# adamjorr/kbbq-py

Measured on NVIDIA B200. Metric: bases/sec recalibrated (table build + apply), higher is better.
Workload: dtype u8 in/out, u32->int64 counts, f64 model

## Files before the change

include/kbbq_b200.h:

```cpp
#ifndef KBBQ_B200_H
#define KBBQ_B200_H

#include <stddef.h>
#include <stdint.h>

#ifdef __cplusplus
extern "C" {
#endif

#define KBBQ_NQ 43
#define KBBQ_NDINUC 16

#define KBBQ_OK 0
#define KBBQ_E_ARG (-1)
#define KBBQ_E_CUDA (-2)
#define KBBQ_E_WORKSPACE (-3)
#define KBBQ_E_DATA (-4)
#define KBBQ_E_IO (-5)
#define KBBQ_E_FORMAT (-6)
#define KBBQ_E_RAGGED (-7)
#define KBBQ_E_NAME_FIELD (-8)
#define KBBQ_E_NAME_RG (-9)
#define KBBQ_E_NAME_MISMATCH (-10)
#define KBBQ_E_PEER (-11)
#define KBBQ_E_UNSUPPORTED (-12)

#define KBBQ_FLAG_QUAL_RANGE 1
#define KBBQ_FLAG_BAD_BASE 2
#define KBBQ_FLAG_RG_RANGE 4
#define KBBQ_FLAG_SEGMENTS 8
#define KBBQ_FLAG_KMER_FULL 16

int kbbq_abi_version(void);
const char *kbbq_strerror(int code);
const char *kbbq_last_cuda_error(void);

int64_t kbbq_pos_table_elems(int L, int R);
int64_t kbbq_din_table_elems(int R);

int kbbq_workspace_bytes(int64_t N, int L, int R, size_t *bytes);

int kbbq_build(const uint8_t *seq_dev, const uint8_t *qual_dev, const uint8_t *corr_dev,
               const uint16_t *rg_dev, const uint8_t *second_dev, int64_t N, int L, int R,
               int minscore, int64_t *pos_errs_dev, int64_t *pos_total_dev, int64_t *din_errs_dev,
               int64_t *din_total_dev, void *workspace_dev, size_t workspace_bytes,
               int *status_dev, int path, void *stream);

int kbbq_marginals(const int64_t *pos_errs_dev, const int64_t *pos_total_dev, int L, int R,
                   int64_t *q_errs_dev, int64_t *q_total_dev, int64_t *rg_errs_dev,
                   int64_t *rg_total_dev, int64_t *meanq_dev, void *stream);

int kbbq_delta_q(const int64_t *prior_q_dev, const int64_t *numerrs_dev,
                 const int64_t *numtotal_dev, int64_t n, int64_t *delta_dev, void *stream);

int kbbq_posterior_q_real(const double *prior_q_dev, const int64_t *numerrs_dev,
                          const int64_t *numtotal_dev, int64_t n, int64_t *posterior_dev, void *stream);

int kbbq_bam_workspace_bytes(int64_t N, int L, int R, size_t *bytes);
int kbbq_build_bam(const uint8_t *seq_dev, const uint8_t *qual_dev, const uint8_t *err_dev,
                   const uint8_t *skip_dev, const uint16_t *rg_dev, const uint8_t *flags_dev,
                   const uint16_t *aln_start_dev, const uint16_t *aln_end_dev, int64_t N, int L, int R,
                   int minscore, int64_t *pos_errs_dev, int64_t *pos_total_dev, int64_t *din_errs_dev,
                   int64_t *din_total_dev, void *workspace_dev, size_t workspace_bytes, int *status_dev,
                   void *stream);
int kbbq_apply_bam(const uint8_t *seq_dev, const uint8_t *qual_dev, const uint16_t *rg_dev,
                   const uint8_t *flags_dev, int64_t N, int L, int R, int minscore,
                   const int64_t *meanq_dev, const int64_t *rgdq_dev, const int64_t *qdq_dev,
                   const int64_t *posdq_dev, const int64_t *dindq_dev, int nq, int ndin1,
                   uint8_t *out_qual_dev, void *workspace_dev, size_t workspace_bytes, int *status_dev,
                   void *stream);

int kbbq_calibration_counts(const uint8_t *qual_dev, const uint8_t *err_dev, const uint8_t *seq_dev,
                            const uint8_t *corr_dev, const uint8_t *skip_dev, int64_t n,
                            int64_t *total_dev, int64_t *errs_dev, void *stream);

int kbbq_get_delta_qs(const int64_t *meanq_dev, const int64_t *rg_errs_dev,
                      const int64_t *rg_total_dev, const int64_t *q_errs_dev,
                      const int64_t *q_total_dev, const int64_t *pos_errs_dev,
                      const int64_t *pos_total_dev, const int64_t *din_errs_dev,
                      const int64_t *din_total_dev, int R, int nq, int ncyc, int ndin,
                      int64_t *rgdq_dev, int64_t *qdq_dev, int64_t *posdq_dev, int64_t *dindq_dev,
                      void *stream);

#define KBBQ_APPLY_BASES_CHECKED 0x10
int kbbq_apply(const uint8_t *seq_dev, const uint8_t *qual_dev, const uint16_t *rg_dev,
               const uint8_t *second_dev, int64_t N, int L, int R, int minscore,
               const int64_t *meanq_dev, const int64_t *rgdq_dev, const int64_t *qdq_dev,
               const int64_t *posdq_dev, const int64_t *dindq_dev, int nq, int ndin1,
               uint8_t *out_qual_dev, void *workspace_dev, size_t workspace_bytes, int *status_dev,
               int path, void *stream);

int64_t kbbq_segment_rows_bound(int64_t N, int R);
int64_t kbbq_segment_table_elems(int R);
int kbbq_segmented_supported(int L, int R, int minscore);
int kbbq_segment_plan(const uint16_t *rg_dev, const uint8_t *second_dev, int64_t N, int R, uint32_t *seg_dev,
                      uint32_t *dest_dev, int *status_dev, void *stream);
int kbbq_segment_rows(const uint8_t *src_dev, const uint32_t *dest_dev, int64_t N, int L, uint8_t *dst_segmented_dev,
                      void *stream);
int kbbq_segment_pad(const uint32_t *seg_dev, int R, int L, uint8_t *seq_dev, uint8_t *qual_dev, uint8_t *corr_dev,
                     void *stream);
int kbbq_unsegment_rows(const uint8_t *src_segmented_dev, const uint32_t *dest_dev, int64_t N, int L,
                        int64_t rows_bound, uint8_t *dst_dev, void *stream);
int kbbq_build_segmented(const uint8_t *seq_dev, const uint8_t *qual_dev, const uint8_t *corr_dev,
                         const uint32_t *seg_dev, int64_t rows_bound, int L, int R, int minscore,
                         int64_t *pos_errs_dev, int64_t *pos_total_dev, int64_t *din_errs_dev,
                         int64_t *din_total_dev, void *workspace_dev, size_t workspace_bytes, int *status_dev,
                         void *stream);
int kbbq_apply_segmented(const uint8_t *seq_dev, const uint8_t *qual_dev, const uint32_t *seg_dev, int64_t rows_bound,
                         int L, int R, int minscore, const int64_t *meanq_dev, const int64_t *rgdq_dev,
                         const int64_t *qdq_dev, const int64_t *posdq_dev, const int64_t *dindq_dev, int nq,
                         int ndin1, uint8_t *out_qual_dev, void *workspace_dev, size_t workspace_bytes,
                         int *status_dev, void *stream);
int kbbq_apply_segmented_flags(const uint8_t *seq_dev, const uint8_t *qual_dev, const uint32_t *seg_dev,
                               int64_t rows_bound, int L, int R, int minscore, const int64_t *meanq_dev,
                               const int64_t *rgdq_dev, const int64_t *qdq_dev, const int64_t *posdq_dev,
                               const int64_t *dindq_dev, int nq, int ndin1, uint8_t *out_qual_dev, void *workspace_dev,
                               size_t workspace_bytes, int *status_dev, int flags, void *stream);

int kbbq_recalibrate_host(const uint8_t *seq, const uint8_t *qual, const uint8_t *corr,
                          const uint16_t *rg, const uint8_t *second, int64_t N, int L, int R,
                          int minscore, uint8_t *out_qual, int64_t *tables_host,
                          int64_t *deltas_host, int *status_out, int device);
int kbbq_recalibrate_host_multi(const uint8_t *seq, const uint8_t *qual, const uint8_t *corr,
                                const uint16_t *rg, const uint8_t *second, int64_t N, int L, int R,
                                int minscore, uint8_t *out_qual, int64_t *tables_host,
                                int64_t *deltas_host, int *status_out, const int *devices, int n_dev);

int kbbq_recalibrate_fastq(const char *reads_path, const char *corrected_path, int infer_rg, int minscore, int out_fd,
                           int device, int threads, int64_t *n_reads, int *n_rg, int *status_out);

int kbbq_host_release(int device);
int kbbq_host_last_traffic(int device, int64_t *h2d_bytes, int64_t *d2h_bytes);
int kbbq_host_pack_mode(int host_threads);

typedef struct kbbq_session kbbq_session;
int kbbq_session_create(int device, int L, int R, int minscore, int64_t chunk_reads, int64_t resident_reads_cap,
                        int host_threads, kbbq_session **out);
void kbbq_session_destroy(kbbq_session *s);
int64_t kbbq_session_chunk_reads(const kbbq_session *s);
int kbbq_session_reset(kbbq_session *s);
int kbbq_session_build_chunk(kbbq_session *s, const uint8_t *seq, const uint8_t *qual, const uint8_t *corr,
                             const uint16_t *rg, const uint8_t *second, int64_t n, int keep_resident);
int kbbq_session_build_range(kbbq_session *s, const uint8_t *seq, const uint8_t *qual, const uint8_t *corr,
                             const uint16_t *rg, const uint8_t *second, int64_t n);
int kbbq_session_tables(kbbq_session *s, int64_t *tables_host);
int kbbq_session_set_tables(kbbq_session *s, const int64_t *tables_host);
int kbbq_session_tables_dev(kbbq_session *s, int64_t **tables_dev, int64_t *elems, void **stream);
int kbbq_session_model(kbbq_session *s, int64_t *deltas_host);
int kbbq_session_apply_resident(kbbq_session *s, int64_t chunk, uint8_t *out_qual);
int kbbq_session_apply_chunk(kbbq_session *s, const uint8_t *seq, const uint8_t *qual, const uint16_t *rg,
                             const uint8_t *second, int64_t n, uint8_t *out_qual);
int kbbq_session_flush(kbbq_session *s);
int kbbq_session_sync(kbbq_session *s, int *status_out);
int kbbq_session_traffic(const kbbq_session *s, int64_t *h2d_bytes, int64_t *d2h_bytes);

int kbbq_build_host(const uint8_t *seq, const uint8_t *qual, const uint8_t *corr,
                    const uint16_t *rg, const uint8_t *second, int64_t N, int L, int R,
                    int minscore, int64_t *pos_errs, int64_t *pos_total, int64_t *din_errs,
                    int64_t *din_total, int *status_out, int device);
int kbbq_apply_host(const uint8_t *seq, const uint8_t *qual, const uint16_t *rg,
                    const uint8_t *second, int64_t N, int L, int R, int minscore,
                    const int64_t *meanq, const int64_t *rgdq, const int64_t *qdq,
                    const int64_t *posdq, const int64_t *dindq, int nq, int ndin1,
                    uint8_t *out_qual, int *status_out, int device);
int kbbq_get_delta_qs_host(const int64_t *meanq, const int64_t *rg_errs, const int64_t *rg_total,
                           const int64_t *q_errs, const int64_t *q_total, const int64_t *pos_errs,
                           const int64_t *pos_total, const int64_t *din_errs,
                           const int64_t *din_total, int R, int nq, int ncyc, int ndin,
                           int64_t *rgdq, int64_t *qdq, int64_t *posdq, int64_t *dindq, int device);
int kbbq_delta_q_host(const int64_t *prior_q, const int64_t *numerrs, const int64_t *numtotal,
                      int64_t n, int64_t *delta, int device);
int kbbq_posterior_q_real_host(const double *prior_q, const int64_t *numerrs, const int64_t *numtotal,
                               int64_t n, int64_t *posterior, int device);
int kbbq_build_bam_host(const uint8_t *seq, const uint8_t *qual, const uint8_t *err, const uint8_t *skip,
                        const uint16_t *rg, const uint8_t *flags, const uint16_t *aln_start,
                        const uint16_t *aln_end, int64_t N, int L, int R, int minscore, int64_t *pos_errs,
                        int64_t *pos_total, int64_t *din_errs, int64_t *din_total, int *status_out,
                        int device);
int kbbq_apply_bam_host(const uint8_t *seq, const uint8_t *qual, const uint16_t *rg, const uint8_t *flags,
                        int64_t N, int L, int R, int minscore, const int64_t *meanq, const int64_t *rgdq,
                        const int64_t *qdq, const int64_t *posdq, const int64_t *dindq, int nq, int ndin1,
                        uint8_t *out_qual, int *status_out, int device);
int kbbq_calibration_counts_host(const uint8_t *qual, const uint8_t *err, const uint8_t *seq,
                                 const uint8_t *corr, const uint8_t *skip, int64_t n, int64_t *total,
                                 int64_t *errs, int device);
int kbbq_marginals_host(const int64_t *pos_errs, const int64_t *pos_total, int L, int R,
                        int64_t *q_errs, int64_t *q_total, int64_t *rg_errs, int64_t *rg_total,
                        int64_t *meanq, int device);

int kbbq_synth_reads(uint64_t seed, int64_t first_read, int64_t n, int L, int R,
                     uint8_t *seq_dev, uint8_t *qual_dev, uint8_t *corr_dev, uint16_t *rg_dev,
                     uint8_t *second_dev, void *stream);

#define KBBQ_PLAN_SEGMENTED 0x100
int kbbq_plan_info(int L, int R, int minscore, int arrays, int max_smem, int *out);

typedef struct kbbq_fastq kbbq_fastq;
int kbbq_fastq_open(const char *path, int threads, kbbq_fastq **out);
int kbbq_fastq_open_mem(const void *data, size_t len, int threads, kbbq_fastq **out);
void kbbq_fastq_close(kbbq_fastq *f);
int64_t kbbq_fastq_num_reads(const kbbq_fastq *f);
int kbbq_fastq_read_len(const kbbq_fastq *f);
int kbbq_fastq_pack(const kbbq_fastq *f, int64_t first, int64_t n, uint8_t *seq, uint8_t *qual, int threads);
int kbbq_fastq_name(const kbbq_fastq *f, int64_t i, const char **name, int *len);
int kbbq_fastq_infer(kbbq_fastq *f, int infer_rg, uint16_t *rg, uint8_t *second, int *n_rg, int threads);
int kbbq_fastq_rg_key(const kbbq_fastq *f, int k, const char **key, int *len);
int kbbq_fastq_check_names(const kbbq_fastq *uncorr, const kbbq_fastq *corr, int64_t n, int threads,
                           int64_t *first_bad);
int kbbq_fastq_write(int fd, const kbbq_fastq *f, int64_t first, int64_t n, const uint8_t *out_qual, int threads);
int kbbq_fastq_format_size(const kbbq_fastq *f, int64_t first, int64_t n, int threads, int64_t *bytes);
int kbbq_fastq_format(const kbbq_fastq *f, int64_t first, int64_t n, const uint8_t *out_qual, char *dst,
                      int64_t dst_bytes, int threads);

int kbbq_host_mismatch_bits(const uint8_t *seq, const uint8_t *corr, int64_t n, uint32_t *bits, int threads);
int kbbq_expand_mismatch_bits(const uint8_t *seq_dev, const uint32_t *bits_dev, int64_t n, uint8_t *corr_dev,
                              void *stream);

int kbbq_host_pack_nibbles(const uint8_t *seq, const uint8_t *corr, int64_t n, uint8_t *packed, int threads,
                           int *bad_base);
int kbbq_expand_nibbles(const uint8_t *packed_dev, int64_t n, uint8_t *seq_dev, uint8_t *corr_dev, void *stream);

int kbbq_kmer_table_bytes(int64_t N, int L, int k, uint64_t *capacity, size_t *bytes);
int kbbq_kmer_clear(void *table_dev, uint64_t capacity, void *stream);
int kbbq_kmer_count(const uint8_t *seq_dev, int64_t N, int L, int k, void *table_dev, uint64_t capacity,
                    int *status_dev, void *stream);
int kbbq_kmer_histogram(const void *table_dev, uint64_t capacity, uint64_t *hist_dev, void *stream);
int kbbq_kmer_flag(const uint8_t *seq_dev, int64_t N, int L, int k, const void *table_dev, uint64_t capacity,
                   int min_count, uint32_t *bits_dev, int *status_dev, void *stream);
int kbbq_kmer_min_count(const uint64_t *hist);

int kbbq_kmer_errors_host(const uint8_t *seq, int64_t N, int L, int k, int min_count, uint32_t *bits_out,
                          uint64_t *hist_out, int *min_count_used, int device);
int kbbq_recalibrate_kmer_host(const uint8_t *seq, const uint8_t *qual, const uint16_t *rg, const uint8_t *second,
                               int64_t N, int L, int R, int minscore, int k, int min_count, uint8_t *out_qual,
                               int64_t *tables_host, int64_t *deltas_host, int *min_count_used, int *status_out,
                               int device);

int64_t kbbq_launch_count(void);

#ifdef __cplusplus
}
#endif
#endif
```

kbbq-py_b200/csrc/host_api.cu:

```cuda
#include <algorithm>
#include <atomic>
#include <chrono>
#include <condition_variable>
#include <memory>
#include <mutex>
#include <sched.h>
#include <stdlib.h>
#include <string.h>
#include <sys/mman.h>
#include <sys/stat.h>
#include <fcntl.h>
#include <thread>
#include <unistd.h>
#include <vector>

#include "common.cuh"

using namespace kbbq;

namespace {

#define KBBQ_TRY(x) do { int rc_ = (x); if (rc_) return rc_; } while (0)

constexpr int MAX_DEVICES = 16;
// ... 1103 lines not shown
        if (status_out) *status_out = st;
        return st ? KBBQ_E_DATA : KBBQ_OK;
    }
};

}

extern "C" {

int kbbq_build_host(const uint8_t *seq, const uint8_t *qual, const uint8_t *corr, const uint16_t *rg,
                    const uint8_t *second, int64_t N, int L, int R, int minscore, int64_t *pos_errs,
                    int64_t *pos_total, int64_t *din_errs, int64_t *din_total, int *status_out, int device) {
    if (N < 0 || L < 1 || R < 1 || R > 65535) return KBBQ_E_ARG;
    if (!pos_errs || !pos_total || !din_errs || !din_total || (N > 0 && (!seq || !qual || !corr))) return KBBQ_E_ARG;
    const size_t nb = (size_t)N * L, npos = (size_t)R * NQ * 2 * L * 8, ndin = (size_t)R * NQ * 16 * 8;
    size_t ws_bytes = 0;
    KBBQ_TRY(kbbq_workspace_bytes(N, L, R, &ws_bytes));
    HostCall c(device, true);
    const auto d_seq = c.span(IN, seq, nb);
    const auto d_qual = c.span(IN, qual, nb);
    const auto d_corr = c.span(IN, corr, nb);
    const auto d_rg = c.span(IN, rg, (size_t)N * 2);
    const auto d_sec = c.span(IN, second, (size_t)N);
    const auto pe = c.span(OUT, pos_errs, npos);
    const auto pt = c.span(OUT, pos_total, npos);
    const auto de = c.span(OUT, din_errs, ndin);
    const auto dt = c.span(OUT, din_total, ndin);
    const auto ws = c.scratch(ws_bytes);
    KBBQ_TRY(c.begin());
    KBBQ_TRY(kbbq_build(d_seq, d_qual, d_corr, d_rg, d_sec, N, L, R, minscore, pe, pt, de, dt, ws, ws_bytes, c.status, 0,
                        nullptr));
    return c.finish(status_out);
}

int kbbq_apply_host(const uint8_t *seq, const uint8_t *qual, const uint16_t *rg, const uint8_t *second, int64_t N,
                    int L, int R, int minscore, const int64_t *meanq, const int64_t *rgdq, const int64_t *qdq,
                    const int64_t *posdq, const int64_t *dindq, int nq, int ndin1, uint8_t *out_qual,
                    int *status_out, int device) {
    if (N < 0 || L < 1 || R < 1 || R > 65535 || nq < 1 || nq > NQ || ndin1 < 16 || ndin1 > 64) return KBBQ_E_ARG;
    if (!meanq || !rgdq || !qdq || !posdq || !dindq || (N > 0 && (!seq || !qual || !out_qual))) return KBBQ_E_ARG;
    const size_t nb = (size_t)N * L, n_q = (size_t)R * nq * 8;
    size_t ws_bytes = 0;
    KBBQ_TRY(kbbq_workspace_bytes(N, L, R, &ws_bytes));
    HostCall c(device, true);
    const auto d_seq = c.span(IN, seq, nb);
    const auto d_qual = c.span(IN, qual, nb);
    const auto d_rg = c.span(IN, rg, (size_t)N * 2);
    const auto d_sec = c.span(IN, second, (size_t)N);
    const auto d_meanq = c.span(IN, meanq, (size_t)R * 8);
    const auto d_rgdq = c.span(IN, rgdq, (size_t)R * 8);
    const auto d_qdq = c.span(IN, qdq, n_q);
    const auto d_posdq = c.span(IN, posdq, n_q * 2 * L);
    const auto d_dindq = c.span(IN, dindq, n_q * ndin1);
    const auto d_out = c.span(OUT, out_qual, nb);
    const auto ws = c.scratch(ws_bytes);
    KBBQ_TRY(c.begin());
    KBBQ_TRY(kbbq_apply(d_seq, d_qual, d_rg, d_sec, N, L, R, minscore, d_meanq, d_rgdq, d_qdq, d_posdq, d_dindq, nq,
                        ndin1, d_out, ws, ws_bytes, c.status, 0, nullptr));
    return c.finish(status_out);
}

int kbbq_get_delta_qs_host(const int64_t *meanq, const int64_t *rg_errs, const int64_t *rg_total,
                           const int64_t *q_errs, const int64_t *q_total, const int64_t *pos_errs,
                           const int64_t *pos_total, const int64_t *din_errs, const int64_t *din_total, int R,
                           int nq, int ncyc, int ndin, int64_t *rgdq, int64_t *qdq, int64_t *posdq,
                           int64_t *dindq, int device) {
    if (R < 1 || nq < 1 || ncyc < 0 || ndin < 0) return KBBQ_E_ARG;
    if (!meanq || !rg_errs || !rg_total || !q_errs || !q_total || !rgdq || !qdq) return KBBQ_E_ARG;
    if ((ncyc && (!pos_errs || !pos_total || !posdq)) || !dindq || (ndin && (!din_errs || !din_total)))
        return KBBQ_E_ARG;
    const size_t nr = (size_t)R * 8, n_q = (size_t)R * nq * 8, n_pos = n_q * ncyc, n_din = n_q * ndin;
    HostCall c(device, false);
    const auto d_meanq = c.span(IN, meanq, nr);
    const auto d_rge = c.span(IN, rg_errs, nr);
    const auto d_rgt = c.span(IN, rg_total, nr);
    const auto d_qe = c.span(IN, q_errs, n_q);
    const auto d_qt = c.span(IN, q_total, n_q);
    const auto d_pe = c.span(IN, pos_errs, n_pos);
    const auto d_pt = c.span(IN, pos_total, n_pos);
    const auto d_de = c.span(IN, din_errs, n_din);
    const auto d_dt = c.span(IN, din_total, n_din);
    const auto o_rg = c.span(OUT, rgdq, nr);
    const auto o_q = c.span(OUT, qdq, n_q);
    const auto o_pos = c.span(OUT, posdq, n_pos);
    const auto o_din = c.span(OUT, dindq, n_q * (ndin + 1));
    KBBQ_TRY(c.begin());
    KBBQ_TRY(kbbq_get_delta_qs(d_meanq, d_rge, d_rgt, d_qe, d_qt, d_pe, d_pt, d_de, d_dt, R, nq, ncyc, ndin, o_rg, o_q,
                               o_pos, o_din, nullptr));
    return c.finish();
}

int kbbq_delta_q_host(const int64_t *prior_q, const int64_t *numerrs, const int64_t *numtotal, int64_t n,
                      int64_t *delta, int device) {
    if (n < 0 || (n > 0 && (!prior_q || !numerrs || !numtotal || !delta))) return KBBQ_E_ARG;
    if (n == 0) return KBBQ_OK;
    HostCall c(device, false);
    const auto d_prior = c.span(IN, prior_q, (size_t)n * 8);
    const auto d_errs = c.span(IN, numerrs, (size_t)n * 8);
    const auto d_total = c.span(IN, numtotal, (size_t)n * 8);
    const auto d_delta = c.span(OUT, delta, (size_t)n * 8);
    KBBQ_TRY(c.begin());
    KBBQ_TRY(kbbq_delta_q(d_prior, d_errs, d_total, n, d_delta, nullptr));
    return c.finish();
}

int kbbq_posterior_q_real_host(const double *prior_q, const int64_t *numerrs, const int64_t *numtotal, int64_t n,
                               int64_t *posterior, int device) {
    if (n < 0 || (n > 0 && (!prior_q || !numerrs || !numtotal || !posterior))) return KBBQ_E_ARG;
    if (n == 0) return KBBQ_OK;
    HostCall c(device, false);
    const auto d_prior = c.span(IN, prior_q, (size_t)n * 8);
    const auto d_errs = c.span(IN, numerrs, (size_t)n * 8);
    const auto d_total = c.span(IN, numtotal, (size_t)n * 8);
    const auto d_post = c.span(OUT, posterior, (size_t)n * 8);
    KBBQ_TRY(c.begin());
    KBBQ_TRY(kbbq_posterior_q_real(d_prior, d_errs, d_total, n, d_post, nullptr));
    return c.finish();
}

int kbbq_build_bam_host(const uint8_t *seq, const uint8_t *qual, const uint8_t *err, const uint8_t *skip,
                        const uint16_t *rg, const uint8_t *flags, const uint16_t *aln_start, const uint16_t *aln_end,
                        int64_t N, int L, int R, int minscore, int64_t *pos_errs, int64_t *pos_total,
                        int64_t *din_errs, int64_t *din_total, int *status_out, int device) {
    if (N < 0 || L < 1 || R < 1 || R > 65535) return KBBQ_E_ARG;
    if (!pos_errs || !pos_total || !din_errs || !din_total || (N > 0 && (!seq || !qual || !err))) return KBBQ_E_ARG;
    const size_t nb = (size_t)N * L, npos = (size_t)R * NQ * 2 * L * 8, ndin = (size_t)R * NQ * 16 * 8;
    size_t ws_bytes = 0;
    KBBQ_TRY(kbbq_bam_workspace_bytes(N, L, R, &ws_bytes));
    HostCall c(device, true);
    const auto d_seq = c.span(IN, seq, nb);
    const auto d_qual = c.span(IN, qual, nb);
    const auto d_err = c.span(IN, err, nb);
    const auto d_skip = c.span(IN, skip, nb);
    const auto d_rg = c.span(IN, rg, (size_t)N * 2);
    const auto d_flags = c.span(IN, flags, (size_t)N);
    const auto d_start = c.span(IN, aln_start, (size_t)N * 2);
    const auto d_end = c.span(IN, aln_end, (size_t)N * 2);
    const auto pe = c.span(INOUT, pos_errs, npos);
    const auto pt = c.span(INOUT, pos_total, npos);
    const auto de = c.span(INOUT, din_errs, ndin);
    const auto dt = c.span(INOUT, din_total, ndin);
    const auto ws = c.scratch(ws_bytes);
    KBBQ_TRY(c.begin());
    KBBQ_TRY(kbbq_build_bam(d_seq, d_qual, d_err, d_skip, d_rg, d_flags, d_start, d_end, N, L, R, minscore, pe, pt, de,
                            dt, ws, ws_bytes, c.status, nullptr));
    return c.finish(status_out);
}

int kbbq_apply_bam_host(const uint8_t *seq, const uint8_t *qual, const uint16_t *rg, const uint8_t *flags, int64_t N,
                        int L, int R, int minscore, const int64_t *meanq, const int64_t *rgdq, const int64_t *qdq,
                        const int64_t *posdq, const int64_t *dindq, int nq, int ndin1, uint8_t *out_qual,
                        int *status_out, int device) {
    if (N < 0 || L < 1 || R < 1 || R > 65535 || nq < 1 || ndin1 != 17) return KBBQ_E_ARG;
    if (!meanq || !rgdq || !qdq || !posdq || !dindq || (N > 0 && (!seq || !qual || !out_qual))) return KBBQ_E_ARG;
    const size_t nb = (size_t)N * L, n_q = (size_t)R * nq * 8;
    size_t ws_bytes = 0;
    KBBQ_TRY(kbbq_bam_workspace_bytes(N, L, R, &ws_bytes));
    HostCall c(device, true);
    const auto d_seq = c.span(IN, seq, nb);
    const auto d_qual = c.span(IN, qual, nb);
    const auto d_rg = c.span(IN, rg, (size_t)N * 2);
    const auto d_flags = c.span(IN, flags, (size_t)N);
    const auto d_meanq = c.span(IN, meanq, (size_t)R * 8);
    const auto d_rgdq = c.span(IN, rgdq, (size_t)R * 8);
    const auto d_qdq = c.span(IN, qdq, n_q);
    const auto d_posdq = c.span(IN, posdq, n_q * 2 * L);
    const auto d_dindq = c.span(IN, dindq, n_q * ndin1);
    const auto d_out = c.span(OUT, out_qual, nb);
    const auto ws = c.scratch(ws_bytes);
    KBBQ_TRY(c.begin());
    KBBQ_TRY(kbbq_apply_bam(d_seq, d_qual, d_rg, d_flags, N, L, R, minscore, d_meanq, d_rgdq, d_qdq, d_posdq, d_dindq,
                            nq, ndin1, d_out, ws, ws_bytes, c.status, nullptr));
    return c.finish(status_out);
}

int kbbq_calibration_counts_host(const uint8_t *qual, const uint8_t *err, const uint8_t *seq, const uint8_t *corr,
                                 const uint8_t *skip, int64_t n, int64_t *total, int64_t *errs, int device) {
    if (n < 0 || !total || !errs || (!err && (!seq || !corr)) || (n > 0 && !qual)) return KBBQ_E_ARG;
    HostCall c(device, false);
    const auto d_qual = c.span(IN, qual, (size_t)n);
    const auto d_err = c.span(IN, err, (size_t)n);
    const auto d_seq = c.span(IN, err ? nullptr : seq, (size_t)n);
    const auto d_corr = c.span(IN, err ? nullptr : corr, (size_t)n);
    const auto d_skip = c.span(IN, skip, (size_t)n);
    const auto d_total = c.span(OUT, total, 256 * 8);
    const auto d_errs = c.span(OUT, errs, 256 * 8);
    KBBQ_TRY(c.begin());
    KBBQ_TRY(kbbq_calibration_counts(d_qual, d_err, d_seq, d_corr, d_skip, n, d_total, d_errs, nullptr));
    return c.finish();
}

int kbbq_marginals_host(const int64_t *pos_errs, const int64_t *pos_total, int L, int R, int64_t *q_errs,
                        int64_t *q_total, int64_t *rg_errs, int64_t *rg_total, int64_t *meanq, int device) {
    if (L < 1 || R < 1) return KBBQ_E_ARG;
    if (!pos_errs || !pos_total || !q_errs || !q_total || !rg_errs || !rg_total || !meanq) return KBBQ_E_ARG;
    const size_t npos = (size_t)R * NQ * 2 * L * 8, n_q = (size_t)R * NQ * 8, nr = (size_t)R * 8;
    HostCall c(device, false);
    const auto pe = c.span(IN, pos_errs, npos);
    const auto pt = c.span(IN, pos_total, npos);
    const auto qe = c.span(OUT, q_errs, n_q);
    const auto qt = c.span(OUT, q_total, n_q);
    const auto ge = c.span(OUT, rg_errs, nr);
    const auto gt = c.span(OUT, rg_total, nr);
    const auto mq = c.span(OUT, meanq, nr);
    KBBQ_TRY(c.begin());
    KBBQ_TRY(kbbq_marginals(pe, pt, L, R, qe, qt, ge, gt, mq, nullptr));
    return c.finish();
}

}


namespace {

int kmer_errors_dev(const uint8_t *seq, int64_t N, int L, int k, int min_count, void *table, uint64_t cap,
                    uint64_t *d_hist, uint32_t *bits, int *d_status, uint64_t *hist, int *t, int *status) {
    KBBQ_TRY(kbbq_kmer_clear(table, cap, nullptr));
    KBBQ_TRY(kbbq_kmer_count(seq, N, L, k, table, cap, d_status, nullptr));
    KBBQ_TRY(kbbq_kmer_histogram(table, cap, d_hist, nullptr));
    KBBQ_CUDA(cudaMemcpy(hist, d_hist, 256 * sizeof(uint64_t), cudaMemcpyDeviceToHost));
    KBBQ_CUDA(cudaMemcpy(status, d_status, sizeof(int), cudaMemcpyDeviceToHost));
    if (*status) return KBBQ_E_DATA;
    *t = min_count > 0 ? min_count : kbbq_kmer_min_count(hist);
    return kbbq_kmer_flag(seq, N, L, k, table, cap, *t, bits, d_status, nullptr);
}

}

extern "C" {

int kbbq_kmer_errors_host(const uint8_t *seq, int64_t N, int L, int k, int min_count, uint32_t *bits_out,
                          uint64_t *hist_out, int *min_count_used, int device) {
    if (N < 0 || L < 1 || k < 1 || k > 31 || min_count < 0 || (N > 0 && (!seq || !bits_out))) return KBBQ_E_ARG;
    uint64_t cap = 0;
    size_t table_bytes = 0;
    KBBQ_TRY(kbbq_kmer_table_bytes(N, L, k, &cap, &table_bytes));
    const size_t nb = (size_t)N * L;
    HostCall c(device, true);
    const auto d_seq = c.span(IN, seq, nb);
    const auto d_bits = c.span(OUT, bits_out, (nb + 31) / 32 * 4);
    const auto d_hist = c.scratch(256 * sizeof(uint64_t));
    const auto table = c.scratch(table_bytes);
    bool ok = false;
    KBBQ_TRY(c.fits(&ok));
    if (!ok) return KBBQ_E_UNSUPPORTED;
    KBBQ_TRY(c.begin());
    uint64_t hist[256];
    int t = 0, st = 0;
    KBBQ_TRY(kmer_errors_dev(d_seq, N, L, k, min_count, table, cap, (uint64_t *)(void *)d_hist, d_bits, c.status, hist,
                             &t, &st));
    if (hist_out) memcpy(hist_out, hist, sizeof(hist));
    if (min_count_used) *min_count_used = t;
    return c.finish();
}

int kbbq_recalibrate_kmer_host(const uint8_t *seq, const uint8_t *qual, const uint16_t *rg, const uint8_t *second,
                               int64_t N, int L, int R, int minscore, int k, int min_count, uint8_t *out_qual,
                               int64_t *tables_host, int64_t *deltas_host, int *min_count_used, int *status_out,
                               int device) {
    if (N < 0 || L < 1 || R < 1 || R > 65535 || minscore < 0 || minscore >= NQ || k < 1 || k > 31 || min_count < 0)
        return KBBQ_E_ARG;
    if (N > 0 && (!seq || !qual || !out_qual)) return KBBQ_E_ARG;
    uint64_t cap = 0;
    size_t table_bytes = 0, ws_bytes = 0;
    KBBQ_TRY(kbbq_kmer_table_bytes(N, L, k, &cap, &table_bytes));
    KBBQ_TRY(kbbq_workspace_bytes(N, L, R, &ws_bytes));
    const size_t nb = (size_t)N * L, npos = (size_t)R * NQ * 2 * L, ndin = (size_t)R * NQ * 16;
    const size_t ntab = 2 * npos + 2 * ndin, nmodel = carve_model(nullptr, L, R).elems;
    HostCall c(device, true);
    const auto d_seq = c.span(IN, seq, nb);
    const auto d_qual = c.span(IN, qual, nb);
    const auto d_rg = c.span(IN, rg, (size_t)N * 2);
    const auto d_sec = c.span(IN, second, (size_t)N);
    const auto d_out = c.span(OUT, out_qual, nb);
    const auto d_bits = c.scratch((nb + 31) / 32 * 4);
    const auto d_corr = c.scratch(nb);
    const auto d_hist = c.scratch(256 * sizeof(uint64_t));
    const auto d_tab = c.scratch(ntab * 8);
    const auto d_model = c.scratch(nmodel * 8);
    const auto ws = c.scratch(ws_bytes);
    const auto table = c.scratch(table_bytes);
    bool ok = false;
    KBBQ_TRY(c.fits(&ok));
    if (!ok) return KBBQ_E_UNSUPPORTED;
    KBBQ_TRY(c.begin());
    uint64_t hist[256];
    int t = 0, st = 0;
    const int rc = kmer_errors_dev(d_seq, N, L, k, min_count, table, cap, (uint64_t *)(void *)d_hist,
                                   (uint32_t *)(void *)d_bits, c.status, hist, &t, &st);
    if (rc == KBBQ_E_DATA && status_out) *status_out = st;
    KBBQ_TRY(rc);
    if (min_count_used) *min_count_used = t;
    int64_t *pe = (int64_t *)(void *)d_tab, *pt = pe + npos, *de = pt + npos, *dt = de + ndin;
    const ModelPtrs mp = carve_model((int64_t *)(void *)d_model, L, R);
    uint8_t *corr = (uint8_t *)(void *)d_corr;
    KBBQ_CUDA(cudaMemset(pe, 0, ntab * 8));
    KBBQ_TRY(kbbq_expand_mismatch_bits(d_seq, (uint32_t *)(void *)d_bits, (int64_t)nb, corr, nullptr));
    KBBQ_TRY(kbbq_build(d_seq, d_qual, corr, d_rg, d_sec, N, L, R, minscore, pe, pt, de, dt, ws, ws_bytes, c.status, 0,
                        nullptr));
    KBBQ_TRY(kbbq_marginals(pe, pt, L, R, mp.q_errs, mp.q_total, mp.rg_errs, mp.rg_total, mp.meanq, nullptr));
    KBBQ_TRY(kbbq_get_delta_qs(mp.meanq, mp.rg_errs, mp.rg_total, mp.q_errs, mp.q_total, pe, pt, de, dt, R, NQ, 2 * L,
                               16, mp.rgdq, mp.qdq, mp.posdq, mp.dindq, nullptr));
    KBBQ_TRY(kbbq_apply(d_seq, d_qual, d_rg, d_sec, N, L, R, minscore, mp.meanq, mp.rgdq, mp.qdq, mp.posdq, mp.dindq, NQ,
                        17, d_out, ws, ws_bytes, c.status, KBBQ_APPLY_BASES_CHECKED, nullptr));
    if (tables_host) KBBQ_CUDA(cudaMemcpy(tables_host, pe, ntab * 8, cudaMemcpyDeviceToHost));
    if (deltas_host)
        KBBQ_CUDA(cudaMemcpy(deltas_host, mp.meanq, ((size_t)2 * R + (size_t)R * NQ * (1 + 2 * L + 17)) * 8,
                             cudaMemcpyDeviceToHost));
    return c.finish(status_out);
}

}
```

kbbq-py_b200/csrc/kbbq_b200.cu:

```cuda
#include <algorithm>
#include <mutex>
#include <stdlib.h>
#include <string.h>
#include <vector>

#include "apply.cuh"
#include "bam.cuh"
#include "build.cuh"
#include "calib.cuh"
#include "common.cuh"
#include "expand.cuh"
#include "kmer.cuh"
#include "model.cuh"
#include "prepare.cuh"
#include "segment.cuh"
#include "synth.cuh"

namespace kbbq {

std::atomic<long long> g_launches{0};
char g_last_cuda_error[256] = "";

static std::mutex g_const_mu;
static bool g_const_done[64];

static int upload_constants() {
    int device;
    KBBQ_CUDA(cudaGetDevice(&device));
    std::lock_guard<std::mutex> lock(g_const_mu);
    if (device >= 0 && device < 64 && g_const_done[device]) return KBBQ_OK;
    KBBQ_CUDA(cudaMemcpyToSymbol(c_lnp, KBBQ_LN_P, sizeof(double) * NQ));
    KBBQ_CUDA(cudaMemcpyToSymbol(c_ln1mp, KBBQ_LN_1MP, sizeof(double) * NQ));
    KBBQ_CUDA(cudaMemcpyToSymbol(c_prior, KBBQ_PRIOR, sizeof(double) * NQ));
    KBBQ_CUDA(cudaMemcpyToSymbol(c_p, KBBQ_P, sizeof(double) * NQ));
    KBBQ_CUDA(cudaMemcpyToSymbol(c_bound_hi, KBBQ_BOUND_HI, sizeof(double) * NQ));
    KBBQ_CUDA(cudaMemcpyToSymbol(c_bound_lo, KBBQ_BOUND_LO, sizeof(double) * NQ));
    if (device >= 0 && device < 64) g_const_done[device] = true;
    return KBBQ_OK;
}

static int current_device_info(int *device, int *sms, int *max_smem) {
    KBBQ_CUDA(cudaGetDevice(device));
    static std::atomic<int> s_sms[64], s_smem[64];
    if (*device < 64 && s_sms[*device].load()) {
        *sms = s_sms[*device].load();
        *max_smem = s_smem[*device].load();
        return KBBQ_OK;
    }
    KBBQ_CUDA(cudaDeviceGetAttribute(sms, cudaDevAttrMultiProcessorCount, *device));
    KBBQ_CUDA(cudaDeviceGetAttribute(max_smem, cudaDevAttrMaxSharedMemoryPerBlockOptin, *device));
    if (*sms <= 0) *sms = KBBQ_SM_COUNT_FALLBACK;
    if (*device < 64) { s_smem[*device].store(*max_smem); s_sms[*device].store(*sms); }
    return KBBQ_OK;
}

static bool misaligned(const void *p, size_t a) { return ((uintptr_t)p & (a - 1)) != 0; }

static bool plan_smem(const Geom &g, int narr, int max_smem, TableCfg *tc, StageLayout *sl) {
    const char *e = getenv("KBBQ_KPS");
    const int kmax = e ? std::max(1, std::min(8, atoi(e))) : 4;
    const char *d = getenv("KBBQ_DREP");
    const int dmax = d ? atoi(d) : 32;
    const char *w = getenv("KBBQ_MIN_STAGES");
    const int want = w ? std::max(2, std::min(8, atoi(w))) : 2;
    const char *ms = getenv("KBBQ_MAX_STAGES");
    const int smax = ms ? std::max(want, std::min(MAX_STAGES, atoi(ms))) : MAX_STAGES;
    struct Rule { int in_flight, kmin, drep; };
    const Rule build_rules[] = {{60000, 2, 32}, {40000, 2, 32}, {0, 2, 32}, {40000, 2, 16}, {0, 2, 16},
                                {40000, 1, 32}, {0, 1, 32}, {40000, 1, 16}, {0, 1, 16}, {0, 1, 8}};
    const Rule apply_rules[] = {{40000, 2, 32}, {0, 2, 32}, {40000, 2, 16}, {0, 2, 16},
                                {40000, 1, 32}, {0, 1, 32}, {40000, 1, 16}, {0, 1, 16}, {0, 1, 8}};
    const Rule *rules = narr == 3 ? build_rules : apply_rules;
    const int nrules = narr == 3 ? 10 : 9;
    const char *f = getenv("KBBQ_IN_FLIGHT");
    for (int r = 0; r < nrules; ++r) {
        const int drep = rules[r].drep;
        if (drep > dmax || (drep == 8 && dmax > 8)) continue;
        const int in_flight_min = (r == 0 && f) ? std::max(0, atoi(f)) : rules[r].in_flight;
        for (int k = kmax; k >= rules[r].kmin; --k) {
            if (!g.contig && g.ng * k > 32) continue;
            if (!make_table_cfg(g, k, drep, narr == 2, tc)) return false;
            for (int s = smax; s >= want; --s) {
                if (s % g.nprod) continue;
                *sl = make_stage_layout(g, narr, s, k, tc->table_bytes);
                if (sl->total > max_smem) continue;
                if ((s - 1) * narr * sl->abytes < in_flight_min) break;
                return true;
            }
        }
    }
    return false;
}

static bool plan_kernel(int L, int R, int minscore, int narr, int max_smem, Geom *g, TableCfg *tc, StageLayout *sl,
                        bool segmode = false) {
    int first = 8;
    if (const char *e = getenv("KBBQ_NPROD")) first = std::max(1, std::min(8, atoi(e)));
    const bool single = R == 1 || segmode;
    for (int nprod = (single ? 1 : first); nprod >= 1; nprod >>= 1) {
        if (!make_geom(L, minscore, single, nprod, g, segmode)) return false;
        if (g->row < 65536 && plan_smem(*g, narr, max_smem, tc, sl)) return true;
    }
    return false;
}

static void (*const build_smem_kernels[8])(BuildArgs) = {
    build_smem_kernel<1, true>, build_smem_kernel<2, true>, build_smem_kernel<3, true>, build_smem_kernel<4, true>,
    build_smem_kernel<5, true>, build_smem_kernel<6, true>, build_smem_kernel<7, true>, build_smem_kernel<8, true>};
static void (*const apply_smem_kernels[2][8])(ApplyArgs) = {
    {apply_smem_kernel<1, false>, apply_smem_kernel<2, false>, apply_smem_kernel<3, false>, apply_smem_kernel<4, false>,
     apply_smem_kernel<5, false>, apply_smem_kernel<6, false>, apply_smem_kernel<7, false>, apply_smem_kernel<8, false>},
    {apply_smem_kernel<1, true>, apply_smem_kernel<2, true>, apply_smem_kernel<3, true>, apply_smem_kernel<4, true>,
     apply_smem_kernel<5, true>, apply_smem_kernel<6, true>, apply_smem_kernel<7, true>, apply_smem_kernel<8, true>}};

template <class Args>
static int launch_smem(void (*kern)(Args), const Args &a, int grid, cudaStream_t st) {
    KBBQ_CUDA(cudaFuncSetAttribute(kern, cudaFuncAttributeMaxDynamicSharedMemorySize, a.sl.total));
    kern<<<grid, a.g.threads + 32 * a.g.nprod, a.sl.total, st>>>(a);
    KBBQ_LAUNCHED();
    return KBBQ_OK;
}

struct SmemPlan {
    Geom g;
    TableCfg tc;
    StageLayout sl;
    Workspace w;
    int sms;
    int64_t N;
    bool smem;
};

template <class Generic>
static int plan_and_prepare(int narr, bool aligned, int64_t N, int L, int R, int minscore, const uint16_t *rg,
                            const uint8_t *second, void *workspace, size_t workspace_bytes, int *status, int path,
                            const unsigned int *seg_rows, cudaStream_t st, const Generic &generic, SmemPlan *p) {
    const bool segmode = seg_rows != nullptr;
    int device, max_smem;
    int rc = current_device_info(&device, &p->sms, &max_smem);
    if (rc) return rc;
    p->smem = path != 2 && aligned && plan_kernel(L, R, minscore, narr, max_smem, &p->g, &p->tc, &p->sl, segmode) &&
              (uint64_t)((N + p->g.G - 1) / p->g.G) < 0xFFFFFFFFull;
    if (!p->smem) {
        if (path == 1 || segmode) return KBBQ_E_ARG;
        return generic(0, N, p->sms * 8);
    }
    p->w = carve_workspace(workspace, N, L, R);
    if (!workspace || workspace_bytes < p->w.bytes) return KBBQ_E_WORKSPACE;
    p->N = N;
    if (segmode) {
        seg_prepare_kernel<<<1, 256, 0, st>>>(seg_rows, 2 * R, p->g.G, (unsigned long long)N, p->w.seg, p->w.uni, status);
        KBBQ_LAUNCHED();
        return KBBQ_OK;
    }
    const int64_t tail = (R == 1 && N > p->g.G) ? N % p->g.G : 0;
    if (tail) {
        p->N = N - tail;
        rc = generic(p->N, tail, 1);
        if (rc) return rc;
    }
    return run_prepare(rg, second, p->N, p->g.G, R, p->w, status, p->sms, p->sl.ngs, p->g.gbytes, p->sl.slot, st);
}

template <class Launch>
static int launch_bam_chunks(long long N, int L, const Launch &launch) {
    const unsigned int wmax = (unsigned int)((3 + L + 3) >> 2);
    const long long per = std::max<long long>(1, (long long)(0x7FFFFFFFu / wmax) / 256 * 256);
    for (long long r0 = 0; r0 < N; r0 += per) {
        const long long n = std::min<long long>(per, N - r0);
        launch((unsigned)((n * wmax + BAM_WARPS * 32 - 1) / (BAM_WARPS * 32)), r0, wmax);
        KBBQ_LAUNCHED();
    }
    return KBBQ_OK;
}

}

using namespace kbbq;

extern "C" {

int kbbq_abi_version(void) { return 1; }

const char *kbbq_strerror(int code) {
    switch (code) {
    case KBBQ_OK: return "ok";
    case KBBQ_E_ARG: return "bad argument";
    case KBBQ_E_CUDA: return "CUDA runtime error";
    case KBBQ_E_WORKSPACE: return "workspace too small";
    case KBBQ_E_DATA: return "input data error (see status flags)";
    case KBBQ_E_IO: return "FASTQ file could not be opened, read or written";
    case KBBQ_E_FORMAT: return "malformed FASTQ (4-line records expected)";
    case KBBQ_E_RAGGED: return "reads of unequal length";
    case KBBQ_E_NAME_FIELD: return "read name has no read-group field";
    case KBBQ_E_NAME_RG: return "read-group field does not start with RG";
    case KBBQ_E_NAME_MISMATCH: return "corrected read name does not start with the read name";
    case KBBQ_E_PEER: return "multi-GPU: peer access between the devices is not available";
    case KBBQ_E_UNSUPPORTED: return "not handled by this entry point (use the chunked driver)";
    default: return "unknown error";
    }
}

const char *kbbq_last_cuda_error(void) { return g_last_cuda_error; }

int64_t kbbq_pos_table_elems(int L, int R) { return (int64_t)R * NQ * 2 * L; }
int64_t kbbq_din_table_elems(int R) { return (int64_t)R * NQ * 16; }
int64_t kbbq_launch_count(void) { return g_launches.load(); }

int kbbq_plan_info(int L, int R, int minscore, int arrays, int max_smem, int *out) {
    const bool segmode = (arrays & KBBQ_PLAN_SEGMENTED) != 0;
    arrays &= ~KBBQ_PLAN_SEGMENTED;
    if (!out || L < 1 || R < 1 || (arrays != 2 && arrays != 3)) return KBBQ_E_ARG;
    Geom g;
    TableCfg tc;
    StageLayout sl;
    if (!plan_kernel(L, R, minscore, arrays, max_smem > 0 ? max_smem : 232448, &g, &tc, &sl, segmode))
        return KBBQ_E_ARG;
    const int v[10] = {g.G, g.lanes, g.ng, g.threads, g.nprod, sl.kps, sl.stages, tc.drep, sl.total, tc.table_bytes};
    for (int i = 0; i < 10; ++i) out[i] = v[i];
    return KBBQ_OK;
}

int kbbq_workspace_bytes(int64_t N, int L, int R, size_t *bytes) {
    if (N < 0 || L < 1 || R < 1 || R > 65535 || !bytes) return KBBQ_E_ARG;
    *bytes = carve_workspace(nullptr, N, L, R).bytes;
    return KBBQ_OK;
}

static int build_impl(const uint8_t *seq, const uint8_t *qual, const uint8_t *corr, const uint16_t *rg,
                      const uint8_t *second, int64_t N, int L, int R, int minscore, int64_t *pos_errs,
                      int64_t *pos_total, int64_t *din_errs, int64_t *din_total, void *workspace,
                      size_t workspace_bytes, int *status, int path, void *stream, const unsigned int *seg_rows) {
    if (N < 0 || L < 1 || R < 1 || R > 65535 || minscore < 0 || minscore >= NQ) return KBBQ_E_ARG;
    if (!pos_errs || !pos_total || !din_errs || !din_total || !status) return KBBQ_E_ARG;
    if (N == 0) return KBBQ_OK;
    if (!seq || !qual || !corr) return KBBQ_E_ARG;
    const bool segmode = seg_rows != nullptr;
    cudaStream_t st = (cudaStream_t)stream;
    auto generic = [&](int64_t r0, int64_t n, int grid) {
        BuildGenericArgs a = {seq + r0 * L, qual + r0 * L, corr + r0 * L, rg ? rg + r0 : nullptr,
                              second ? second + r0 : nullptr, n, L, R, minscore,
                              (unsigned long long *)pos_errs, (unsigned long long *)pos_total,
                              (unsigned long long *)din_errs, (unsigned long long *)din_total, status};
        build_generic_kernel<<<grid, 256, 0, st>>>(a);
        KBBQ_LAUNCHED();
        return KBBQ_OK;
    };
    const bool aligned = !misaligned(seq, 16) && !misaligned(qual, 16) && !misaligned(corr, 16);
    SmemPlan p;
    int rc = plan_and_prepare(3, aligned, N, L, R, minscore, rg, second, workspace, workspace_bytes, status, path,
                              seg_rows, st, generic, &p);
    if (rc || !p.smem) return rc;

    BuildArgs a;
    a.seq = seq; a.qual = qual; a.corr = corr; a.total_bytes = p.N * L; a.g = p.g; a.t = p.tc; a.R = R;
    a.nsub = segmode ? 2 * R : R; a.segmode = segmode ? 1 : 0;
    a.sl = p.sl;
    a.entries = p.w.entries; a.seg = p.w.seg; a.uni = p.w.uni;
    a.pos_errs = (unsigned long long *)pos_errs; a.pos_total = (unsigned long long *)pos_total;
    a.din_errs = (unsigned long long *)din_errs; a.din_total = (unsigned long long *)din_total;
    a.status = status;
    return launch_smem(build_smem_kernels[a.sl.kps - 1], a, p.sms, st);
}

int kbbq_build(const uint8_t *seq, const uint8_t *qual, const uint8_t *corr, const uint16_t *rg,
               const uint8_t *second, int64_t N, int L, int R, int minscore, int64_t *pos_errs,
               int64_t *pos_total, int64_t *din_errs, int64_t *din_total, void *workspace,
               size_t workspace_bytes, int *status, int path, void *stream) {
    return build_impl(seq, qual, corr, rg, second, N, L, R, minscore, pos_errs, pos_total, din_errs, din_total,
                      workspace, workspace_bytes, status, path, stream, nullptr);
}

int kbbq_build_segmented(const uint8_t *seq, const uint8_t *qual, const uint8_t *corr, const uint32_t *seg,
                         int64_t rows_bound, int L, int R, int minscore, int64_t *pos_errs, int64_t *pos_total,
                         int64_t *din_errs, int64_t *din_total, void *workspace, size_t workspace_bytes, int *status,
                         void *stream) {
    if (!seg || rows_bound % SEG_ALIGN) return KBBQ_E_ARG;
    return build_impl(seq, qual, corr, nullptr, nullptr, rows_bound, L, R, minscore, pos_errs, pos_total, din_errs,
                      din_total, workspace, workspace_bytes, status, 1, stream, seg);
}

int kbbq_marginals(const int64_t *pos_errs, const int64_t *pos_total, int L, int R, int64_t *q_errs,
                   int64_t *q_total, int64_t *rg_errs, int64_t *rg_total, int64_t *meanq, void *stream) {
    if (L < 1 || R < 1 || !pos_errs || !pos_total || !q_errs || !q_total || !rg_errs || !rg_total || !meanq)
        return KBBQ_E_ARG;
    cudaStream_t st = (cudaStream_t)stream;
    int rc = upload_constants();
    if (rc) return rc;
    marginals_q_kernel<<<dim3(NQ, R), 128, 0, st>>>((const long long *)pos_errs, (const long long *)pos_total,
                                                   2 * L, (long long *)q_errs, (long long *)q_total);
    KBBQ_LAUNCHED();
    marginals_rg_kernel<<<R, 64, 0, st>>>((const long long *)q_errs, (const long long *)q_total, R,
                                                      (long long *)rg_errs, (long long *)rg_total, (long long *)meanq);
    KBBQ_LAUNCHED();
    return KBBQ_OK;
}

int kbbq_delta_q(const int64_t *prior_q, const int64_t *numerrs, const int64_t *numtotal, int64_t n,
                 int64_t *delta, void *stream) {
    if (n < 0 || (n > 0 && (!prior_q || !numerrs || !numtotal || !delta))) return KBBQ_E_ARG;
    if (n == 0) return KBBQ_OK;
    int rc = upload_constants();
    if (rc) return rc;
    delta_q_kernel<<<(unsigned)((n + 127) / 128), 128, 0, (cudaStream_t)stream>>>(
        (const long long *)prior_q, (const long long *)numerrs, (const long long *)numtotal, n, (long long *)delta);
    KBBQ_LAUNCHED();
    return KBBQ_OK;
}

int kbbq_posterior_q_real(const double *prior_q, const int64_t *numerrs, const int64_t *numtotal, int64_t n,
                          int64_t *posterior, void *stream) {
    if (n < 0 || (n > 0 && (!prior_q || !numerrs || !numtotal || !posterior))) return KBBQ_E_ARG;
    if (n == 0) return KBBQ_OK;
    int rc = upload_constants();
    if (rc) return rc;
    posterior_q_real_kernel<<<(unsigned)((n + 127) / 128), 128, 0, (cudaStream_t)stream>>>(
        prior_q, (const long long *)numerrs, (const long long *)numtotal, n, (long long *)posterior);
    KBBQ_LAUNCHED();
    return KBBQ_OK;
}

struct BamWorkspace {
    uint8_t *cseq, *cqual, *cthird, *csecond;
    void *inner;
    size_t inner_bytes, bytes;
};
static BamWorkspace carve_bam_workspace(void *base, long long N, int L, int R) {
    BamWorkspace w = {};
    char *p = (char *)base;
    size_t off = 0;
    const size_t nb = align_up((size_t)N * L + 16, 256);
    w.cseq = (uint8_t *)(p + off); off += nb;
    w.cqual = (uint8_t *)(p + off); off += nb;
    w.cthird = (uint8_t *)(p + off); off += nb;
    w.csecond = (uint8_t *)(p + off); off += align_up((size_t)N + 16, 256);
    w.inner = p + off;
    w.inner_bytes = carve_workspace(nullptr, N, L, R).bytes;
    w.bytes = off + w.inner_bytes;
    return w;
}

int kbbq_bam_workspace_bytes(int64_t N, int L, int R, size_t *bytes) {
    if (N < 0 || L < 1 || R < 1 || R > 65535 || !bytes) return KBBQ_E_ARG;
    *bytes = carve_bam_workspace(nullptr, N, L, R).bytes;
    return KBBQ_OK;
}

int kbbq_build_bam(const uint8_t *seq, const uint8_t *qual, const uint8_t *err, const uint8_t *skip, const uint16_t *rg,
                   const uint8_t *flags, const uint16_t *aln_start, const uint16_t *aln_end, int64_t N, int L, int R,
                   int minscore, int64_t *pos_errs, int64_t *pos_total, int64_t *din_errs, int64_t *din_total,
                   void *workspace, size_t workspace_bytes, int *status, void *stream) {
    if (N < 0 || L < 1 || L > 32767 || R < 1 || R > 65535 || minscore < 0 || minscore >= NQ) return KBBQ_E_ARG;
    if (!pos_errs || !pos_total || !din_errs || !din_total || !status) return KBBQ_E_ARG;
    if (N == 0) return KBBQ_OK;
    if (!seq || !qual || !err) return KBBQ_E_ARG;
    int device, sms, max_smem;
    int rc = current_device_info(&device, &sms, &max_smem);
    if (rc) return rc;
    cudaStream_t st = (cudaStream_t)stream;
    const long long blocks = std::min<long long>(((long long)N * L + 255) / 256, (long long)sms * 16);
    if (workspace && minscore >= 1) {
        BamWorkspace w = carve_bam_workspace(workspace, N, L, R);
        if (workspace_bytes < w.bytes) return KBBQ_E_WORKSPACE;
        BamCanonArgs c = {seq, qual, err, skip, rg, flags, aln_start, aln_end, N, L, R, minscore, NQ, true,
                          w.cseq, w.cqual, w.cthird, w.csecond,
                          (unsigned long long *)pos_errs, (unsigned long long *)pos_total,
                          (unsigned long long *)din_errs, (unsigned long long *)din_total, status};
        rc = launch_bam_chunks(N, L, [&](unsigned grid, long long r0, unsigned wmax) {
            bam_canon_kernel<<<grid, BAM_WARPS * 32, 0, st>>>(c, r0, wmax);
        });
        if (rc) return rc;
        return kbbq_build(w.cseq, w.cqual, w.cthird, rg, w.csecond, N, L, R, minscore, pos_errs, pos_total, din_errs,
                          din_total, w.inner, w.inner_bytes, status, 0, stream);
    }
    BuildBamArgs a = {seq, qual, err, skip, rg, flags, aln_start, aln_end, N, L, R, minscore,
                      (unsigned long long *)pos_errs, (unsigned long long *)pos_total,
                      (unsigned long long *)din_errs, (unsigned long long *)din_total, status};
    build_bam_kernel<<<(unsigned)blocks, 256, 0, st>>>(a);
    KBBQ_LAUNCHED();
    return KBBQ_OK;
}

int kbbq_apply_bam(const uint8_t *seq, const uint8_t *qual, const uint16_t *rg, const uint8_t *flags, int64_t N, int L,
                   int R, int minscore, const int64_t *meanq, const int64_t *rgdq, const int64_t *qdq,
                   const int64_t *posdq, const int64_t *dindq, int nq, int ndin1, uint8_t *out_qual, void *workspace,
                   size_t workspace_bytes, int *status, void *stream) {
    if (N < 0 || L < 1 || L > 32767 || R < 1 || R > 65535 || minscore < 0 || minscore >= NQ || nq < 1 || nq > 256 ||
        ndin1 != 17)
        return KBBQ_E_ARG;
    if (!meanq || !rgdq || !qdq || !posdq || !dindq || !status) return KBBQ_E_ARG;
    if (N == 0) return KBBQ_OK;
    if (!seq || !qual || !out_qual) return KBBQ_E_ARG;
    int device, sms, max_smem;
    int rc = current_device_info(&device, &sms, &max_smem);
    if (rc) return rc;
    cudaStream_t st = (cudaStream_t)stream;
    const long long blocks = std::min<long long>(((long long)N * L + 255) / 256, (long long)sms * 16);
    if (workspace && minscore >= 1 && nq <= NQ) {
        BamWorkspace w = carve_bam_workspace(workspace, N, L, R);
        if (workspace_bytes < w.bytes) return KBBQ_E_WORKSPACE;
        BamCanonArgs c = {seq, qual, nullptr, nullptr, rg, flags, nullptr, nullptr, N, L, R, minscore, nq, false,
                          w.cseq, w.cqual, nullptr, w.csecond, nullptr, nullptr, nullptr, nullptr, status};
        rc = launch_bam_chunks(N, L, [&](unsigned grid, long long r0, unsigned wmax) {
            bam_canon_kernel<<<grid, BAM_WARPS * 32, 0, st>>>(c, r0, wmax);
        });
        if (rc) return rc;
        rc = kbbq_apply(w.cseq, w.cqual, rg, w.csecond, N, L, R, minscore, meanq, rgdq, qdq, posdq, dindq, nq, ndin1,
                        w.cthird, w.inner, w.inner_bytes, status, KBBQ_APPLY_BASES_CHECKED, stream);
        if (rc) return rc;
        return launch_bam_chunks(N, L, [&](unsigned grid, long long r0, unsigned wmax) {
            bam_uncanon_kernel<<<grid, BAM_WARPS * 32, 0, st>>>(w.cthird, flags, N, L, out_qual, r0, wmax);
        });
    }
    ApplyBamArgs a = {seq, qual, rg, flags, out_qual, N, L, R, minscore, nq, ndin1, (const long long *)meanq,
                      (const long long *)rgdq, (const long long *)qdq, (const long long *)posdq,
                      (const long long *)dindq, status};
    apply_bam_kernel<<<(unsigned)blocks, 256, 0, st>>>(a);
    KBBQ_LAUNCHED();
    return KBBQ_OK;
}

int kbbq_calibration_counts(const uint8_t *qual, const uint8_t *err, const uint8_t *seq, const uint8_t *corr,
                            const uint8_t *skip, int64_t n, int64_t *total, int64_t *errs, void *stream) {
    if (n < 0 || !total || !errs) return KBBQ_E_ARG;
    if (n == 0) return KBBQ_OK;
    if (!qual || (!err && (!seq || !corr))) return KBBQ_E_ARG;
    cudaStream_t st = (cudaStream_t)stream;
    int device, sms, max_smem;
    int rc = current_device_info(&device, &sms, &max_smem);
    if (rc) return rc;
    auto misaligned = [](const void *p) { return p && ((uintptr_t)p & 15u); };
    CalibArgs a = {qual, err, seq, corr, skip, n, (unsigned long long *)total, (unsigned long long *)errs};
    if (misaligned(qual) || misaligned(err) || misaligned(skip) || (!err && (misaligned(seq) || misaligned(corr)))) {
        const long long chunk = 1ll << 31;
        for (long long o = 0; o < n; o += chunk) {
            CalibArgs c = a;
            c.qual += o; if (err) c.err += o; else { c.seq += o; c.corr += o; } if (skip) c.skip += o;
            c.n = std::min<long long>(chunk, n - o);
            calibration_scalar_kernel<<<sms * 8, CAL_THREADS, 0, st>>>(c);
            KBBQ_LAUNCHED();
        }
        return KBBQ_OK;
    }
    const int grid = sms * 3;
    const long long chunk = (long long)grid * CAL_THREADS * CAL_MAX_ITERS * 32;
    auto kern = err ? (skip ? calibration_kernel<true, true> : calibration_kernel<true, false>)
                    : (skip ? calibration_kernel<false, true> : calibration_kernel<false, false>);
    KBBQ_CUDA(cudaFuncSetAttribute(kern, cudaFuncAttributeMaxDynamicSharedMemorySize, CAL_SMEM));
    for (long long o = 0; o < n; o += chunk) {
        CalibArgs c = a;
        c.qual += o; if (err) c.err += o; else { c.seq += o; c.corr += o; } if (skip) c.skip += o;
        c.n = std::min<long long>(chunk, n - o);
        kern<<<grid, CAL_THREADS, CAL_SMEM, st>>>(c);
        KBBQ_LAUNCHED();
    }
    return KBBQ_OK;
}

int kbbq_get_delta_qs(const int64_t *meanq, const int64_t *rg_errs, const int64_t *rg_total,
                      const int64_t *q_errs, const int64_t *q_total, const int64_t *pos_errs,
                      const int64_t *pos_total, const int64_t *din_errs, const int64_t *din_total, int R,
                      int nq, int ncyc, int ndin, int64_t *rgdq, int64_t *qdq, int64_t *posdq,
                      int64_t *dindq, void *stream) {
    if (R < 1 || nq < 1 || ncyc < 0 || ndin < 0) return KBBQ_E_ARG;
    if (!meanq || !rg_errs || !rg_total || !q_errs || !q_total || !rgdq || !qdq) return KBBQ_E_ARG;
    if ((ncyc && (!pos_errs || !pos_total || !posdq)) || !dindq || (ndin && (!din_errs || !din_total)))
        return KBBQ_E_ARG;
    int rc = upload_constants();
    if (rc) return rc;
    cudaStream_t st = (cudaStream_t)stream;
    DeltaArgs a = {(const long long *)meanq, (const long long *)rg_errs, (const long long *)rg_total,
                   (const long long *)q_errs, (const long long *)q_total, (const long long *)pos_errs,
                   (const long long *)pos_total, (const long long *)din_errs, (const long long *)din_total,
                   R, nq, ncyc, ndin, (long long *)rgdq, (long long *)qdq, (long long *)posdq, (long long *)dindq};
    delta_levels12_kernel<<<R, 64, 0, st>>>(a);
    KBBQ_LAUNCHED();
    const long long cells = (long long)R * nq * (ncyc + ndin + 1);
    delta_level3_kernel<<<(unsigned)((cells + 127) / 128), 128, 0, st>>>(a);
    KBBQ_LAUNCHED();
    return KBBQ_OK;
}

static int apply_impl(const uint8_t *seq, const uint8_t *qual, const uint16_t *rg, const uint8_t *second, int64_t N,
                      int L, int R, int minscore, const int64_t *meanq, const int64_t *rgdq, const int64_t *qdq,
                      const int64_t *posdq, const int64_t *dindq, int nq, int ndin1, uint8_t *out_qual,
                      void *workspace, size_t workspace_bytes, int *status, int path, void *stream,
                      const unsigned int *seg_rows) {
    const bool segmode = seg_rows != nullptr;
    const bool validate = !(path & KBBQ_APPLY_BASES_CHECKED);
    path &= ~KBBQ_APPLY_BASES_CHECKED;
    if (N < 0 || L < 1 || R < 1 || R > 65535 || minscore < 0 || minscore >= NQ) return KBBQ_E_ARG;
    if (nq < 1 || nq > NQ || ndin1 < 16 || ndin1 > 64) return KBBQ_E_ARG;
    if (!meanq || !rgdq || !qdq || !posdq || !dindq || !status) return KBBQ_E_ARG;
    if (N == 0) return KBBQ_OK;
    if (!seq || !qual || !out_qual) return KBBQ_E_ARG;
    cudaStream_t st = (cudaStream_t)stream;
    Workspace w = carve_workspace(workspace, N, L, R);
    if (!workspace || workspace_bytes < w.bytes) return KBBQ_E_WORKSPACE;

    const long long fold_cells = (long long)R * NQ * (2 * L + 16);
    fold_kernel<<<(unsigned)((fold_cells + 255) / 256), 256, 0, st>>>(
        (const long long *)meanq, (const long long *)rgdq, (const long long *)qdq, (const long long *)posdq,
        (const long long *)dindq, R, nq, 2 * L, ndin1, w.fold_cyc, w.fold_din);
    KBBQ_LAUNCHED();

    auto generic = [&](int64_t r0, int64_t n, int grid) {
        ApplyGenericArgs a = {seq + r0 * L, qual + r0 * L, rg ? rg + r0 : nullptr, second ? second + r0 : nullptr,
                              out_qual + r0 * L, n, L, R, minscore, nq, w.fold_cyc, w.fold_din, status, validate};
        apply_generic_kernel<<<grid, 256, 0, st>>>(a);
        KBBQ_LAUNCHED();
        return KBBQ_OK;
    };
    const bool aligned = !misaligned(seq, 16) && !misaligned(qual, 16) && !misaligned(out_qual, 4);
    SmemPlan p;
    int rc = plan_and_prepare(2, aligned, N, L, R, minscore, rg, second, workspace, workspace_bytes, status, path,
                              seg_rows, st, generic, &p);
    if (rc || !p.smem) return rc;

    ApplyArgs a;
    a.nsub = segmode ? 2 * R : R; a.segmode = segmode ? 1 : 0;
    a.seq = seq; a.qual = qual; a.out = out_qual; a.total_bytes = p.N * L; a.g = p.g; a.t = p.tc; a.R = R; a.nq = nq;
    a.sl = p.sl;
    a.entries = w.entries; a.seg = w.seg; a.uni = w.uni; a.fold_cyc = w.fold_cyc; a.fold_din = w.fold_din; a.status = status;
    return launch_smem(apply_smem_kernels[validate][a.sl.kps - 1], a, p.sms, st);
}

int kbbq_apply(const uint8_t *seq, const uint8_t *qual, const uint16_t *rg, const uint8_t *second, int64_t N,
               int L, int R, int minscore, const int64_t *meanq, const int64_t *rgdq, const int64_t *qdq,
               const int64_t *posdq, const int64_t *dindq, int nq, int ndin1, uint8_t *out_qual,
               void *workspace, size_t workspace_bytes, int *status, int path, void *stream) {
    return apply_impl(seq, qual, rg, second, N, L, R, minscore, meanq, rgdq, qdq, posdq, dindq, nq, ndin1, out_qual,
                      workspace, workspace_bytes, status, path, stream, nullptr);
}

int kbbq_apply_segmented_flags(const uint8_t *seq, const uint8_t *qual, const uint32_t *seg, int64_t rows_bound, int L,
                               int R, int minscore, const int64_t *meanq, const int64_t *rgdq, const int64_t *qdq,
                               const int64_t *posdq, const int64_t *dindq, int nq, int ndin1, uint8_t *out_qual,
                               void *workspace, size_t workspace_bytes, int *status, int flags, void *stream) {
    if (!seg || rows_bound % SEG_ALIGN || (flags & ~KBBQ_APPLY_BASES_CHECKED)) return KBBQ_E_ARG;
    return apply_impl(seq, qual, nullptr, nullptr, rows_bound, L, R, minscore, meanq, rgdq, qdq, posdq, dindq, nq, ndin1,
                      out_qual, workspace, workspace_bytes, status, 1 | flags, stream, seg);
}

int kbbq_apply_segmented(const uint8_t *seq, const uint8_t *qual, const uint32_t *seg, int64_t rows_bound, int L, int R,
                         int minscore, const int64_t *meanq, const int64_t *rgdq, const int64_t *qdq,
                         const int64_t *posdq, const int64_t *dindq, int nq, int ndin1, uint8_t *out_qual,
                         void *workspace, size_t workspace_bytes, int *status, void *stream) {
    return kbbq_apply_segmented_flags(seq, qual, seg, rows_bound, L, R, minscore, meanq, rgdq, qdq, posdq, dindq, nq, ndin1,
                                      out_qual, workspace, workspace_bytes, status, 0, stream);
}


int64_t kbbq_segment_rows_bound(int64_t N, int R) {
    if (N < 0 || R < 1) return -1;
    return (N + SEG_ALIGN - 1) / SEG_ALIGN * SEG_ALIGN + (int64_t)2 * R * SEG_ALIGN;
}

int64_t kbbq_segment_table_elems(int R) { return R < 1 ? -1 : (int64_t)6 * R + 1; }

int kbbq_segmented_supported(int L, int R, int minscore) {
    if (L < 1 || R < 1 || R > 65535) return 0;
    Geom g;
    TableCfg tc;
    StageLayout sl;
    return plan_kernel(L, R, minscore, 3, 232448, &g, &tc, &sl, true) && plan_kernel(L, R, minscore, 2, 232448, &g, &tc, &sl, true);
}

int kbbq_segment_plan(const uint16_t *rg, const uint8_t *second, int64_t N, int R, uint32_t *seg, uint32_t *dest,
                      int *status, void *stream) {
    if (N < 0 || R < 1 || R > 65535 || !seg || !status || (N > 0 && !dest)) return KBBQ_E_ARG;
    if (kbbq_segment_rows_bound(N, R) >= 0xFFFFFFFFll) return KBBQ_E_ARG;
    cudaStream_t st = (cudaStream_t)stream;
    const int nkeys = 2 * R;
    SegPlanArgs a = {rg, second, N, R, seg, seg + 2 * nkeys + 1, dest, status};
    KBBQ_CUDA(cudaMemsetAsync(a.cursor, 0, sizeof(unsigned int) * nkeys, st));
    const int per_thread = 8;
    const long long per_block = (long long)SEG_THREADS * per_thread;
    const unsigned int blocks = (unsigned int)((N + per_block - 1) / per_block);
    const size_t smem = nkeys <= SEG_SMEM_KEYS ? sizeof(unsigned int) * nkeys : 0;
    if (blocks) {
        seg_bucket_kernel<0><<<blocks, SEG_THREADS, smem, st>>>(a, per_thread);
        KBBQ_LAUNCHED();
    }
    seg_scan_kernel<<<1, 1024, 0, st>>>(a);
    KBBQ_LAUNCHED();
    if (blocks) {
        seg_bucket_kernel<1><<<blocks, SEG_THREADS, smem, st>>>(a, per_thread);
        KBBQ_LAUNCHED();
    }
    return KBBQ_OK;
}

static int move_rows(const uint8_t *src, const uint32_t *dest, int64_t N, int L, uint8_t *dst, int64_t src_rows, bool scatter,
                     cudaStream_t st) {
    if (N < 0 || L < 1 || src_rows < 0) return KBBQ_E_ARG;
    if (N == 0) return KBBQ_OK;
    if (!src || !dest || !dst) return KBBQ_E_ARG;
    int device, sms, max_smem;
    int rc = current_device_info(&device, &sms, &max_smem);
    if (rc) return rc;
    const long long warps_per_block = SEG_THREADS / 32;
    const unsigned int blocks = (unsigned int)std::min<long long>((N + warps_per_block - 1) / warps_per_block, (long long)sms * 32);
    if (scatter) seg_move_rows_kernel<true><<<blocks, SEG_THREADS, 0, st>>>(src, dst, dest, N, L, src_rows);
    else seg_move_rows_kernel<false><<<blocks, SEG_THREADS, 0, st>>>(src, dst, dest, N, L, src_rows);
    KBBQ_LAUNCHED();
    return KBBQ_OK;
}

int kbbq_segment_rows(const uint8_t *src, const uint32_t *dest, int64_t N, int L, uint8_t *dst_segmented, void *stream) {
    return move_rows(src, dest, N, L, dst_segmented, N, true, (cudaStream_t)stream);
}

int kbbq_unsegment_rows(const uint8_t *src_segmented, const uint32_t *dest, int64_t N, int L, int64_t rows_bound,
                        uint8_t *dst, void *stream) {
    return move_rows(src_segmented, dest, N, L, dst, rows_bound, false, (cudaStream_t)stream);
}

int kbbq_segment_pad(const uint32_t *seg, int R, int L, uint8_t *seq, uint8_t *qual, uint8_t *corr, void *stream) {
    if (!seg || R < 1 || R > 65535 || L < 1) return KBBQ_E_ARG;
    seg_pad_kernel<<<2 * R, 128, 0, (cudaStream_t)stream>>>(seg, 2 * R, L, seq, qual, corr);
    KBBQ_LAUNCHED();
    return KBBQ_OK;
}

int kbbq_synth_reads(uint64_t seed, int64_t first_read, int64_t n, int L, int R, uint8_t *seq, uint8_t *qual,
                     uint8_t *corr, uint16_t *rg, uint8_t *second, void *stream) {
    if (n < 0 || L < 1 || R < 1 || R > 65535 || first_read < 0) return KBBQ_E_ARG;
    if (n == 0) return KBBQ_OK;
    if (!seq || !qual || !corr) return KBBQ_E_ARG;
    int device, sms, max_smem;
    int rc = current_device_info(&device, &sms, &max_smem);
    if (rc) return rc;
    synth_kernel<<<sms * 16, 256, 0, (cudaStream_t)stream>>>(seed, first_read, n, L, R, seq, qual, corr, rg, second);
    KBBQ_LAUNCHED();
    return KBBQ_OK;
}

int kbbq_expand_mismatch_bits(const uint8_t *seq, const uint32_t *bits, int64_t n, uint8_t *corr, void *stream) {
    if (n < 0 || (n > 0 && (!seq || !bits || !corr))) return KBBQ_E_ARG;
    if (n == 0) return KBBQ_OK;
    if (((uintptr_t)seq | (uintptr_t)corr) & 15u) return KBBQ_E_ARG;
    expand_corr_kernel<<<(unsigned)((n + 16 * 256 - 1) / (16 * 256)), 256, 0, (cudaStream_t)stream>>>(seq, bits, corr, n);
    KBBQ_LAUNCHED();
    return KBBQ_OK;
}

int kbbq_expand_nibbles(const uint8_t *packed, int64_t n, uint8_t *seq, uint8_t *corr, void *stream) {
    if (n < 0 || (n > 0 && (!packed || !seq || !corr))) return KBBQ_E_ARG;
    if (n == 0) return KBBQ_OK;
    if (((uintptr_t)packed | (uintptr_t)seq | (uintptr_t)corr) & 15u) return KBBQ_E_ARG;
    expand_nibbles_kernel<<<(unsigned)((n + 32 * 256 - 1) / (32 * 256)), 256, 0, (cudaStream_t)stream>>>(packed, seq, corr, n);
    KBBQ_LAUNCHED();
    return KBBQ_OK;
}


static bool kmer_table_ok(const void *table, uint64_t capacity) {
    return table && !misaligned(table, 16) && capacity >= 1 && (capacity & (capacity - 1)) == 0;
}

int kbbq_kmer_table_bytes(int64_t N, int L, int k, uint64_t *capacity, size_t *bytes) {
    if (N < 0 || L < 1 || k < 1 || k > 31 || !capacity) return KBBQ_E_ARG;
    const uint64_t windows = (uint64_t)N * (uint64_t)std::max(0, L - k + 1);
    const uint64_t need = windows + (windows + 1) / 2;
    if (need > (1ull << 59)) return KBBQ_E_ARG;
    uint64_t cap = 1;
    while (cap < need) cap <<= 1;
    *capacity = cap;
    if (bytes) *bytes = (size_t)(cap * 16);
    return KBBQ_OK;
}

int kbbq_kmer_clear(void *table, uint64_t capacity, void *stream) {
    if (!kmer_table_ok(table, capacity)) return KBBQ_E_ARG;
    int device, sms, max_smem;
    int rc = current_device_info(&device, &sms, &max_smem);
    if (rc) return rc;
    const uint64_t blocks = std::min<uint64_t>((capacity + 255) / 256, (uint64_t)sms * 16);
    kmer_clear_kernel<<<(unsigned)blocks, 256, 0, (cudaStream_t)stream>>>((ulonglong2 *)table, capacity);
    KBBQ_LAUNCHED();
    return KBBQ_OK;
}

int kbbq_kmer_count(const uint8_t *seq, int64_t N, int L, int k, void *table, uint64_t capacity, int *status,
                    void *stream) {
    if (N < 0 || L < 1 || k < 1 || k > 31 || !status || !kmer_table_ok(table, capacity)) return KBBQ_E_ARG;
    if (N == 0 || L < k) return KBBQ_OK;
    if (!seq) return KBBQ_E_ARG;
    kmer_count_kernel<<<(unsigned)((N + 255) / 256), 256, 0, (cudaStream_t)stream>>>(
        seq, N, L, k, (unsigned long long *)table, capacity - 1, status);
    KBBQ_LAUNCHED();
    return KBBQ_OK;
}

int kbbq_kmer_histogram(const void *table, uint64_t capacity, uint64_t *hist, void *stream) {
    if (!kmer_table_ok(table, capacity) || !hist) return KBBQ_E_ARG;
    int device, sms, max_smem;
    int rc = current_device_info(&device, &sms, &max_smem);
    if (rc) return rc;
    KBBQ_CUDA(cudaMemsetAsync(hist, 0, 256 * sizeof(uint64_t), (cudaStream_t)stream));
    const uint64_t blocks = std::min<uint64_t>((capacity + 255) / 256, (uint64_t)sms * 8);
    kmer_hist_kernel<<<(unsigned)blocks, 256, 0, (cudaStream_t)stream>>>((const ulonglong2 *)table, capacity,
                                                                         (unsigned long long *)hist);
    KBBQ_LAUNCHED();
    return KBBQ_OK;
}

int kbbq_kmer_flag(const uint8_t *seq, int64_t N, int L, int k, const void *table, uint64_t capacity, int min_count,
                   uint32_t *bits, int *status, void *stream) {
    if (N < 0 || L < 1 || k < 1 || k > 31 || min_count < 1 || !status || !kmer_table_ok(table, capacity))
        return KBBQ_E_ARG;
    if (N == 0) return KBBQ_OK;
    if (!seq || !bits) return KBBQ_E_ARG;
    int device, sms, max_smem;
    int rc = current_device_info(&device, &sms, &max_smem);
    if (rc) return rc;
    const int warps = std::max(1, std::min(4, 49152 / (4 * L)));
    const size_t smem = (size_t)warps * L * 4;
    if (smem > (size_t)max_smem) return KBBQ_E_ARG;
    if (smem > 49152) KBBQ_CUDA(cudaFuncSetAttribute(kmer_flag_kernel, cudaFuncAttributeMaxDynamicSharedMemorySize, (int)smem));
    const int64_t blocks = (N + 32 * warps - 1) / (32 * warps);
    kmer_flag_kernel<<<(unsigned)blocks, 32 * warps, smem, (cudaStream_t)stream>>>(
        seq, N, L, k, (const ulonglong2 *)table, capacity - 1, (unsigned long long)min_count, bits, status);
    KBBQ_LAUNCHED();
    return KBBQ_OK;
}

int kbbq_kmer_min_count(const uint64_t *hist) {
    if (!hist) return KBBQ_E_ARG;
    for (int c = 2; c <= 254; ++c)
        if (hist[c] <= hist[c + 1]) return c;
    return 255;
}

}
```

kbbq-py_b200/csrc/model.cuh:

```cuda
#pragma once
#include "common.cuh"

namespace kbbq {

__constant__ double c_lnp[NQ];
__constant__ double c_ln1mp[NQ];
__constant__ double c_prior[NQ];
__constant__ double c_p[NQ];
__constant__ double c_bound_hi[NQ];
__constant__ double c_bound_lo[NQ];

struct dd { double hi, lo; };
__device__ __forceinline__ dd two_sum(double a, double b) {
    double s = __dadd_rn(a, b), bb = __dsub_rn(s, a);
    double e = __dadd_rn(__dsub_rn(a, __dsub_rn(s, bb)), __dsub_rn(b, bb));
    return {s, e};
}
__device__ __forceinline__ dd two_prod(double a, double b) {
    double p = __dmul_rn(a, b);
    return {p, __fma_rn(a, b, -p)};
}
__device__ __forceinline__ dd dd_add(dd a, dd b) {
    dd s = two_sum(a.hi, b.hi);
    double lo = __dadd_rn(s.lo, __dadd_rn(a.lo, b.lo));
    return two_sum(s.hi, lo);
}
__device__ __forceinline__ dd dd_div_d(dd a, double b) {
    double q1 = __ddiv_rn(a.hi, b);
    dd p = two_prod(q1, b);
    double r = __dadd_rn(__dsub_rn(__dsub_rn(a.hi, p.hi), p.lo), a.lo);
    double q2 = __ddiv_rn(r, b);
    return two_sum(q1, q2);
}
__device__ __forceinline__ bool dd_le(dd a, double bh, double bl) {
    return a.hi < bh || (a.hi == bh && a.lo <= bl);
}

__global__ void marginals_q_kernel(const long long *pos_errs, const long long *pos_total, int L2,
                                   long long *q_errs, long long *q_total) {
    const int q = blockIdx.x, rg = blockIdx.y;
    const size_t base = ((size_t)rg * NQ + q) * L2;
    long long e = 0, t = 0;
    for (int c = threadIdx.x; c < L2; c += blockDim.x) { e += pos_errs[base + c]; t += pos_total[base + c]; }
    __shared__ long long se[32], st[32];
    for (int o = 16; o; o >>= 1) { e += __shfl_down_sync(0xFFFFFFFFu, e, o); t += __shfl_down_sync(0xFFFFFFFFu, t, o); }
    if ((threadIdx.x & 31) == 0) { se[threadIdx.x >> 5] = e; st[threadIdx.x >> 5] = t; }
    __syncthreads();
    if (threadIdx.x == 0) {
        e = 0; t = 0;
        for (int w = 0; w < (blockDim.x + 31) / 32; ++w) { e += se[w]; t += st[w]; }
        q_errs[rg * NQ + q] = e;
        q_total[rg * NQ + q] = t;
    }
}

__global__ void marginals_rg_kernel(const long long *q_errs, const long long *q_total, int R,
                                    long long *rg_errs, long long *rg_total, long long *meanq) {
    const int rg = blockIdx.x;
    __shared__ long long s_e[NQ], s_t[NQ];
    if (threadIdx.x < NQ) {
        s_e[threadIdx.x] = q_errs[rg * NQ + threadIdx.x];
        s_t[threadIdx.x] = q_total[rg * NQ + threadIdx.x];
    }
    __syncthreads();
    if (threadIdx.x != 0) return;
    long long e = 0, t = 0;
    dd acc = {0.0, 0.0};
    for (int q = 0; q < NQ; ++q) {
        const long long tq = s_t[q];
        e += s_e[q];
        t += tq;
        if (tq) acc = dd_add(acc, two_prod((double)tq, c_p[q]));
    }
    rg_errs[rg] = e;
    rg_total[rg] = t;
    long long mq = 0;
    if (t > 0) {
        if (acc.hi == 0.0) mq = NQ - 1;
        else {
            const dd p = dd_div_d(acc, (double)t);
            for (int m = 1; m < NQ; ++m) mq += dd_le(p, c_bound_hi[m], c_bound_lo[m]) ? 1 : 0;
        }
    }
    meanq[rg] = mq;
}

__device__ __forceinline__ dd round_to_x87(dd s) {
    if (s.lo == 0.0 || isinf(s.hi) || isnan(s.hi)) return s;
    int e;
    frexp(s.hi, &e);
    int eh = e - 1;
    if (fabs(s.hi) == ldexp(1.0, eh) && ((s.hi > 0.0) != (s.lo > 0.0))) eh -= 1;
    const int qe = eh - 63;
    const double lo_r = ldexp(rint(ldexp(s.lo, -qe)), qe);
    const double h = __dadd_rn(s.hi, lo_r);
    return {h, __dadd_rn(__dsub_rn(s.hi, h), lo_r)};
}

template <typename PRIOR>
__device__ __forceinline__ int posterior_q_cell(PRIOR prior, long long errs, long long tot) {
    const double k = (double)(errs + 1), mm = (double)((tot + 2) - (errs + 1));
    int best = 0;
    double bh = 0.0, bl = 0.0;
    bool have = false;
    for (int c = 0; c < NQ; ++c) {
        int d = (int)((PRIOR)c - prior);
        d = d < 0 ? -d : d;
        const double pr = d < NQ ? c_prior[d] : -KBBQ_INF;
        const double a = __dmul_rn(k, c_lnp[c]);
        const double b = (mm == 0.0) ? 0.0 : __dmul_rn(mm, c_ln1mp[c]);
        const double ll = __dadd_rn(a, b);
        double h, l;
        if (isinf(pr) || isinf(ll)) { h = -KBBQ_INF; l = 0.0; }
        else { dd s = round_to_x87(two_sum(pr, ll)); h = s.hi; l = s.lo; }
        if (!have || h > bh || (h == bh && l > bl)) { best = c; bh = h; bl = l; have = true; }
    }
    return best;
}
__device__ __forceinline__ int delta_q_cell(int prior, long long errs, long long tot) {
    return posterior_q_cell<int>(prior, errs, tot) - prior;
}

__global__ void delta_q_kernel(const long long *prior, const long long *errs, const long long *tot,
                               long long n, long long *out) {
    long long i = (long long)blockIdx.x * blockDim.x + threadIdx.x;
    if (i < n) out[i] = delta_q_cell((int)prior[i], errs[i], tot[i]);
}

__global__ void posterior_q_real_kernel(const double *prior, const long long *errs, const long long *tot,
                                        long long n, long long *out) {
    long long i = (long long)blockIdx.x * blockDim.x + threadIdx.x;
    if (i < n) out[i] = posterior_q_cell<double>(prior[i], errs[i], tot[i]);
}

struct DeltaArgs {
    const long long *meanq, *rg_errs, *rg_total, *q_errs, *q_total, *pos_errs, *pos_total, *din_errs, *din_total;
    int R, nq, ncyc, ndin;
    long long *rgdq, *qdq, *posdq, *dindq;
};

__global__ void delta_levels12_kernel(DeltaArgs a) {
    const int rg = blockIdx.x;
    __shared__ int s_prior1;
    if (threadIdx.x == 0) {
        const int mq = (int)a.meanq[rg];
        const int d = delta_q_cell(mq, a.rg_errs[rg], a.rg_total[rg]);
        a.rgdq[rg] = d;
        s_prior1 = mq + d;
    }
    __syncthreads();
    for (int q = threadIdx.x; q < a.nq; q += blockDim.x)
        a.qdq[rg * a.nq + q] = delta_q_cell(s_prior1, a.q_errs[rg * a.nq + q], a.q_total[rg * a.nq + q]);
}

__global__ void delta_level3_kernel(DeltaArgs a) {
    const long long ncell_pos = (long long)a.R * a.nq * a.ncyc;
    const long long ncell_din = (long long)a.R * a.nq * (a.ndin + 1);
    long long i = (long long)blockIdx.x * blockDim.x + threadIdx.x;
    if (i < ncell_pos) {
        const long long gq = i / a.ncyc;
        const int rg = (int)(gq / a.nq);
        const int prior2 = (int)(a.meanq[rg] + a.rgdq[rg] + a.qdq[gq]);
        a.posdq[i] = delta_q_cell(prior2, a.pos_errs[i], a.pos_total[i]);
    } else if (i < ncell_pos + ncell_din) {
        i -= ncell_pos;
        const long long gq = i / (a.ndin + 1);
        const int d = (int)(i - gq * (a.ndin + 1));
        if (d == a.ndin) { a.dindq[i] = 0; return; }
        const int rg = (int)(gq / a.nq);
        const int prior2 = (int)(a.meanq[rg] + a.rgdq[rg] + a.qdq[gq]);
        a.dindq[i] = delta_q_cell(prior2, a.din_errs[gq * a.ndin + d], a.din_total[gq * a.ndin + d]);
    }
}

__global__ void fold_kernel(const long long *meanq, const long long *rgdq, const long long *qdq,
                            const long long *posdq, const long long *dindq, int R, int nq, int L2,
                            int ndin1, short *fold_cyc, short *fold_din) {
    const long long ncyc = (long long)R * NQ * L2, ndin = (long long)R * NQ * 16;
    long long i = (long long)blockIdx.x * blockDim.x + threadIdx.x;
    if (i < ncyc) {
        const long long gq = i / L2;
        const int c2 = (int)(i - gq * L2);
        const int rg = (int)(gq / NQ), q = (int)(gq - (long long)rg * NQ);
        long long v = 0;
        if (q < nq)
            v = meanq[rg] + rgdq[rg] + qdq[rg * nq + q] + posdq[((size_t)rg * nq + q) * L2 + c2] +
                dindq[((size_t)rg * nq + q) * ndin1 + ndin1 - 1];
        fold_cyc[i] = (short)v;
    } else if (i < ncyc + ndin) {
        i -= ncyc;
        const long long gq = i >> 4;
        const int n = (int)(i & 15);
        const int rg = (int)(gq / NQ), q = (int)(gq - (long long)rg * NQ);
        long long v = 0;
        if (q < nq) {
            const size_t row = ((size_t)rg * nq + q) * ndin1;
            v = dindq[row + nat_to_ref(n >> 2) * 4 + nat_to_ref(n & 3)] - dindq[row + ndin1 - 1];
        }
        fold_din[i] = (short)v;
    }
}

}
```

kbbq-py_b200/csrc/prepare.cuh:

```cuda
#pragma once
#include "common.cuh"

namespace kbbq {

constexpr int PREP_THREADS = 256;
constexpr int PREP_SMEM_RG = 8192;

struct PrepArgs {
    const uint16_t *rg;
    const uint8_t *second;
    long long N;
    long long ngroups;
    int G;
    int R;
    unsigned int *seg;
    unsigned int *cursor;
    entry_t *entries;
    unsigned int *uni;
    int *status;
    int grid;
    int ng;
    unsigned int gbytes;
    unsigned int slot;
};

__device__ __forceinline__ entry_t make_entry(unsigned int soff, long long grp, unsigned int match, unsigned int sec) {
    unsigned int f[2] = {0u, 0u};
#pragma unroll
    for (int k = 0; k < MAX_G; ++k) {
        const unsigned int live = (match >> k) & 1u, s2 = (sec >> k) & 1u;
        f[k >> 2] |= (live | ((live & s2) << 1)) << (8 * (k & 3));
    }
    return make_uint4(soff, (unsigned int)grp, f[0], f[1]);
}

__device__ __forceinline__ unsigned long long slice_lo(unsigned long long E, unsigned long long b, int grid) {
    return E * b / (unsigned long long)grid;
}
__device__ __forceinline__ unsigned long long slice_of(unsigned long long E, unsigned long long i, int grid) {
    return ((i + 1) * (unsigned long long)grid + E - 1) / E - 1;
}

__device__ __forceinline__ void load_rows(const PrepArgs &a, long long grp, unsigned int rgv[MAX_G],
                                          unsigned int &sec, unsigned int &exist) {
    sec = 0;
    exist = 0;
#pragma unroll
    for (int k = 0; k < MAX_G; ++k) {
        rgv[k] = 0xFFFFFFFFu;
        if (k < a.G) {
            const long long r = grp * a.G + k;
            if (r < a.N) {
                rgv[k] = a.rg ? a.rg[r] : 0u;
                exist |= 1u << k;
                if (a.second && a.second[r]) sec |= 1u << k;
            }
        }
    }
}

__device__ __forceinline__ void identity_rows(const PrepArgs &a, long long grp, unsigned int &exist, unsigned int &sec,
                                              bool report) {
    unsigned int rgv[MAX_G];
    load_rows(a, grp, rgv, sec, exist);
    if (a.rg) {
        unsigned int ok = 0;
#pragma unroll
        for (int k = 0; k < MAX_G; ++k)
            if ((exist >> k) & 1) {
                if (rgv[k] == 0) ok |= 1u << k;
                else if (report) atomicOr(a.status, KBBQ_FLAG_RG_RANGE);
            }
        exist = ok;
    }
}

__global__ void prep_uniform_kernel(PrepArgs a) {
    const long long t0 = (long long)blockIdx.x * blockDim.x + threadIdx.x;
    const long long stride = (long long)gridDim.x * blockDim.x;
    if (t0 == 0) {
        a.seg[0] = 0;
        a.seg[1] = (unsigned int)a.ngroups;
    }
    unsigned int exist0, sec0;
    identity_rows(a, 0, exist0, sec0, false);
    bool differs = exist0 != (1u << a.G) - 1u;
    for (int k = 2; k < a.G; ++k) differs |= ((sec0 >> k) & 1u) != ((sec0 >> (k & 1)) & 1u);
    const bool wide = (a.G & (a.G - 1)) == 0 && a.G <= 16 && (!a.second || ((uintptr_t)a.second & 15u) == 0) &&
                      (!a.rg || ((uintptr_t)a.rg & 15u) == 0);
    long long done_groups = 0;
    if (wide) {
        const long long chunks = a.N / 16;
        uint4 pat;
        {
            unsigned int v[4];
            for (int j = 0; j < 4; ++j) {
                v[j] = 0;
                for (int k = 0; k < 4; ++k) v[j] |= ((sec0 >> ((4 * j + k) % a.G)) & 1u) << (8 * k);
            }
            pat = make_uint4(v[0], v[1], v[2], v[3]);
        }
        for (long long c = t0; c < chunks; c += stride) {
            if (a.second) {
                const uint4 s = reinterpret_cast<const uint4 *>(a.second)[c];
                auto norm = [](unsigned int x) { return ((x | ((x | 0x80808080u) - 0x01010101u)) >> 7) & 0x01010101u; };
                differs |= norm(s.x) != pat.x || norm(s.y) != pat.y || norm(s.z) != pat.z || norm(s.w) != pat.w;
            } else {
                differs |= sec0 != 0;
            }
            if (a.rg) {
                const uint4 r0 = reinterpret_cast<const uint4 *>(a.rg)[2 * c], r1 = reinterpret_cast<const uint4 *>(a.rg)[2 * c + 1];
                if (r0.x | r0.y | r0.z | r0.w | r1.x | r1.y | r1.z | r1.w) { differs = true; atomicOr(a.status, KBBQ_FLAG_RG_RANGE); }
            }
        }
        done_groups = chunks * 16 / a.G;
    }
    for (long long grp = done_groups + t0; grp < a.ngroups; grp += stride) {
        unsigned int exist, sec;
        identity_rows(a, grp, exist, sec, true);
        differs |= exist != exist0 || sec != sec0;
    }
    if (differs) a.uni[0] = 1u;
    if (t0 == 0) {
        const entry_t p0 = make_entry(0u, 0, exist0, sec0);
        a.uni[1] = p0.z;
        a.uni[2] = p0.w;
    }
}

__global__ void prep_identity_kernel(PrepArgs a) {
    if (a.uni[0] == 0u) return;
    const unsigned long long E = (unsigned long long)a.ngroups;
    for (long long grp = (long long)blockIdx.x * blockDim.x + threadIdx.x; grp < a.ngroups;
         grp += (long long)gridDim.x * blockDim.x) {
        unsigned int exist, sec;
        identity_rows(a, grp, exist, sec, false);
        const unsigned long long lo = slice_lo(E, slice_of(E, (unsigned long long)grp, a.grid), a.grid);
        const unsigned int j = (unsigned int)(((unsigned long long)grp - lo) % (unsigned int)a.ng);
        const unsigned int mis0 = (unsigned int)((((unsigned long long)grp - j) * a.gbytes) & 15ull);
        a.entries[grp] = make_entry(mis0 + j * a.gbytes, grp, exist, sec);
    }
}

template <int MODE>
__global__ void __launch_bounds__(PREP_THREADS) prep_bucket_kernel(PrepArgs a) {
    extern __shared__ unsigned int s_cnt[];
    const bool use_smem = a.R <= PREP_SMEM_RG;
    if (use_smem) {
        for (int i = threadIdx.x; i < a.R; i += blockDim.x) s_cnt[i] = 0;
        __syncthreads();
    }
    const long long grp = (long long)blockIdx.x * blockDim.x + threadIdx.x;
    unsigned int rgv[MAX_G], exist = 0, sec = 0;
    unsigned int slot[MAX_G], mask[MAX_G];
    if (grp < a.ngroups) load_rows(a, grp, rgv, sec, exist);
#pragma unroll
    for (int k = 0; k < MAX_G; ++k) {
        mask[k] = 0;
        slot[k] = 0;
        if (!((exist >> k) & 1)) continue;
        const unsigned int v = rgv[k];
        if (v >= (unsigned int)a.R) {
            atomicOr(a.status, KBBQ_FLAG_RG_RANGE);
            continue;
        }
        bool first = true;
        unsigned int m = 0;
#pragma unroll
        for (int k2 = 0; k2 < MAX_G; ++k2) {
            if (((exist >> k2) & 1) && rgv[k2] == v) {
                if (k2 < k) first = false;
                m |= 1u << k2;
            }
        }
        if (!first) continue;
        mask[k] = m;
        if (use_smem) slot[k] = atomicAdd(&s_cnt[v], 1u);
        else slot[k] = atomicAdd(&a.cursor[v], 1u);
    }
    if (use_smem) {
        __syncthreads();
        for (int i = threadIdx.x; i < a.R; i += blockDim.x) {
            const unsigned int c = s_cnt[i];
            if (c) s_cnt[i] = atomicAdd(&a.cursor[i], c);
        }
        if (MODE == 0) return;
        __syncthreads();
    }
    if (MODE == 1) {
        const unsigned long long E = a.seg[a.R];
#pragma unroll
        for (int k = 0; k < MAX_G; ++k) {
            if (!mask[k]) continue;
            const unsigned int pos = slot[k] + (use_smem ? s_cnt[rgv[k]] : 0u);
            const unsigned long long lo = slice_lo(E, slice_of(E, pos, a.grid), a.grid);
            const unsigned long long start = max((unsigned long long)a.seg[rgv[k]], lo);
            const unsigned int j = (unsigned int)((pos - start) % (unsigned int)a.ng);
            const unsigned int mis = (unsigned int)(((unsigned long long)grp * a.gbytes) & 15ull);
            a.entries[pos] = make_entry(j * a.slot + mis, grp, mask[k], sec);
        }
    }
}

__global__ void prep_scan_kernel(PrepArgs a) {
    __shared__ unsigned int s_part[1024];
    const int T = blockDim.x;
    const int per = (a.R + T - 1) / T;
    const int lo = threadIdx.x * per, hi = min(a.R, lo + per);
    unsigned int sum = 0;
    for (int i = lo; i < hi; ++i) sum += a.cursor[i];
    s_part[threadIdx.x] = sum;
    __syncthreads();
    if (threadIdx.x == 0) {
        unsigned int run = 0;
        for (int t = 0; t < T; ++t) {
            const unsigned int v = s_part[t];
            s_part[t] = run;
            run += v;
        }
        a.seg[a.R] = run;
    }
    __syncthreads();
    unsigned int run = s_part[threadIdx.x];
    for (int i = lo; i < hi; ++i) {
        const unsigned int v = a.cursor[i];
        a.seg[i] = run;
        a.cursor[i] = run;
        run += v;
    }
}

struct Workspace {
    unsigned int *seg;
    unsigned int *cursor;
    unsigned int *uni;
    entry_t *entries;
    short *fold_cyc;
    short *fold_din;
    size_t bytes;
};

inline size_t align_up(size_t v, size_t a) { return (v + a - 1) / a * a; }

inline Workspace carve_workspace(void *base, long long N, int L, int R) {
    Workspace w = {};
    size_t off = 0;
    char *p = (char *)base;
    const size_t max_entries = (size_t)N + MAX_G;
    w.seg = (unsigned int *)(p + off);      off = align_up(off + sizeof(unsigned int) * (2 * (size_t)R + 2), 256);
    w.cursor = (unsigned int *)(p + off);   off = align_up(off + sizeof(unsigned int) * (size_t)R, 256);
    w.uni = (unsigned int *)(p + off);      off = align_up(off + sizeof(unsigned int) * 4, 256);
    w.entries = (entry_t *)(p + off);       off = align_up(off + sizeof(entry_t) * max_entries, 256);
    w.fold_cyc = (short *)(p + off);        off = align_up(off + sizeof(short) * (size_t)R * NQ * 2 * L, 256);
    w.fold_din = (short *)(p + off);        off = align_up(off + sizeof(short) * (size_t)R * NQ * 16, 256);
    w.bytes = off;
    return w;
}

inline int run_prepare(const uint16_t *rg, const uint8_t *second, long long N, int G, int R,
                       const Workspace &w, int *status, int grid, int ng, unsigned int gbytes,
                       unsigned int slot, cudaStream_t st) {
    PrepArgs a;
    a.rg = rg; a.second = second; a.N = N; a.G = G;
    a.ngroups = (N + G - 1) / G; a.R = R;
    a.seg = w.seg; a.cursor = w.cursor; a.entries = w.entries; a.uni = w.uni; a.status = status;
    a.grid = grid; a.ng = ng; a.gbytes = gbytes; a.slot = slot;
    KBBQ_CUDA(cudaMemsetAsync(w.uni, (R == 1 && a.ngroups > 0) ? 0 : 0xFF, sizeof(unsigned int) * 4, st));
    if (a.ngroups == 0) {
        KBBQ_CUDA(cudaMemsetAsync(w.seg, 0, sizeof(unsigned int) * ((size_t)R + 1), st));
        return KBBQ_OK;
    }
    const unsigned int blocks = (unsigned int)((a.ngroups + PREP_THREADS - 1) / PREP_THREADS);
    if (R == 1) {
        const unsigned int few = std::min<unsigned int>(blocks, (unsigned int)std::max(grid, 1) * 8u);
        prep_uniform_kernel<<<few, PREP_THREADS, 0, st>>>(a);
        KBBQ_LAUNCHED();
        prep_identity_kernel<<<few, PREP_THREADS, 0, st>>>(a);
        KBBQ_LAUNCHED();
        return KBBQ_OK;
    }
    const size_t smem = R <= PREP_SMEM_RG ? sizeof(unsigned int) * (size_t)R : 0;
    KBBQ_CUDA(cudaMemsetAsync(w.cursor, 0, sizeof(unsigned int) * (size_t)R, st));
    prep_bucket_kernel<0><<<blocks, PREP_THREADS, smem, st>>>(a);
    KBBQ_LAUNCHED();
    prep_scan_kernel<<<1, 1024, 0, st>>>(a);
    KBBQ_LAUNCHED();
    prep_bucket_kernel<1><<<blocks, PREP_THREADS, smem, st>>>(a);
    KBBQ_LAUNCHED();
    return KBBQ_OK;
}

}
```

kbbq-py_b200/kbbq/_native.py:

```python
import ctypes as C
import os

import numpy as np

HERE = os.path.dirname(os.path.abspath(__file__))
LIB_PATH = os.path.join(HERE, "libkbbq_b200.so")

NQ = 43
FLAG_QUAL_RANGE, FLAG_BAD_BASE, FLAG_RG_RANGE, FLAG_SEGMENTS = 1, 2, 4, 8
FLAG_KMER_FULL = 16
APPLY_BASES_CHECKED = 0x10
E_DATA = -4
E_UNSUPPORTED = -12

_lib = None

_vp, _i, _i64, _sz = C.c_void_p, C.c_int, C.c_int64, C.c_size_t
SIGNATURES = {
    "kbbq_abi_version": (_i, []),
    "kbbq_strerror": (C.c_char_p, [_i]),
    "kbbq_last_cuda_error": (C.c_char_p, []),
    "kbbq_pos_table_elems": (_i64, [_i, _i]),
    "kbbq_din_table_elems": (_i64, [_i]),
    "kbbq_workspace_bytes": (_i, [_i64, _i, _i, C.POINTER(_sz)]),
    "kbbq_build": (_i, [_vp] * 5 + [_i64, _i, _i, _i] + [_vp] * 4 + [_vp, _sz, _vp, _i, _vp]),
    "kbbq_marginals": (_i, [_vp, _vp, _i, _i] + [_vp] * 5 + [_vp]),
    "kbbq_delta_q": (_i, [_vp, _vp, _vp, _i64, _vp, _vp]),
    "kbbq_get_delta_qs": (_i, [_vp] * 9 + [_i, _i, _i, _i] + [_vp] * 4 + [_vp]),
    "kbbq_apply": (_i, [_vp] * 4 + [_i64, _i, _i, _i] + [_vp] * 5 + [_i, _i, _vp, _vp, _sz, _vp, _i, _vp]),
    "kbbq_recalibrate_host": (_i, [_vp] * 5 + [_i64, _i, _i, _i] + [_vp] * 3 + [C.POINTER(_i), _i]),
    "kbbq_recalibrate_host_multi": (_i, [_vp] * 5 + [_i64, _i, _i, _i] + [_vp] * 3 + [C.POINTER(_i), C.POINTER(_i), _i]),
    "kbbq_recalibrate_fastq": (_i, [C.c_char_p, C.c_char_p, _i, _i, _i, _i, _i, C.POINTER(_i64), C.POINTER(_i), C.POINTER(_i)]),
    "kbbq_host_release": (_i, [_i]),
    "kbbq_session_create": (_i, [_i, _i, _i, _i, _i64, _i64, _i, C.POINTER(_vp)]),
    "kbbq_session_destroy": (None, [_vp]),
    "kbbq_session_chunk_reads": (_i64, [_vp]),
    "kbbq_session_reset": (_i, [_vp]),
    "kbbq_session_build_chunk": (_i, [_vp] * 6 + [_i64, _i]),
    "kbbq_session_build_range": (_i, [_vp] * 6 + [_i64]),
    "kbbq_session_tables": (_i, [_vp, _vp]),
    "kbbq_session_set_tables": (_i, [_vp, _vp]),
    "kbbq_session_tables_dev": (_i, [_vp, C.POINTER(_vp), C.POINTER(_i64), C.POINTER(_vp)]),
    "kbbq_session_model": (_i, [_vp, _vp]),
    "kbbq_session_apply_resident": (_i, [_vp, _i64, _vp]),
    "kbbq_session_apply_chunk": (_i, [_vp] * 5 + [_i64, _vp]),
    "kbbq_session_flush": (_i, [_vp]),
    "kbbq_session_sync": (_i, [_vp, C.POINTER(_i)]),
    "kbbq_session_traffic": (_i, [_vp, C.POINTER(_i64), C.POINTER(_i64)]),
    "kbbq_build_host": (_i, [_vp] * 5 + [_i64, _i, _i, _i] + [_vp] * 4 + [C.POINTER(_i), _i]),
    "kbbq_apply_host": (_i, [_vp] * 4 + [_i64, _i, _i, _i] + [_vp] * 5 + [_i, _i, _vp, C.POINTER(_i), _i]),
    "kbbq_get_delta_qs_host": (_i, [_vp] * 9 + [_i, _i, _i, _i] + [_vp] * 4 + [_i]),
    "kbbq_delta_q_host": (_i, [_vp, _vp, _vp, _i64, _vp, _i]),
    "kbbq_posterior_q_real": (_i, [_vp, _vp, _vp, _i64, _vp, _vp]),
    "kbbq_posterior_q_real_host": (_i, [_vp, _vp, _vp, _i64, _vp, _i]),
    "kbbq_calibration_counts": (_i, [_vp] * 5 + [_i64, _vp, _vp, _vp]),
    "kbbq_calibration_counts_host": (_i, [_vp] * 5 + [_i64, _vp, _vp, _i]),
    "kbbq_bam_workspace_bytes": (_i, [_i64, _i, _i, C.POINTER(_sz)]),
    "kbbq_build_bam": (_i, [_vp] * 8 + [_i64, _i, _i, _i] + [_vp] * 4 + [_vp, _sz, _vp, _vp]),
    "kbbq_apply_bam": (_i, [_vp] * 4 + [_i64, _i, _i, _i] + [_vp] * 5 + [_i, _i, _vp, _vp, _sz, _vp, _vp]),
    "kbbq_build_bam_host": (_i, [_vp] * 8 + [_i64, _i, _i, _i] + [_vp] * 4 + [_vp, _i]),
    "kbbq_apply_bam_host": (_i, [_vp] * 4 + [_i64, _i, _i, _i] + [_vp] * 5 + [_i, _i, _vp, _vp, _i]),
    "kbbq_marginals_host": (_i, [_vp, _vp, _i, _i] + [_vp] * 5 + [_i]),
    "kbbq_synth_reads": (_i, [C.c_uint64, _i64, _i64, _i, _i] + [_vp] * 5 + [_vp]),
    "kbbq_launch_count": (_i64, []),
    "kbbq_fastq_open": (_i, [C.c_char_p, _i, C.POINTER(_vp)]),
    "kbbq_fastq_open_mem": (_i, [_vp, _sz, _i, C.POINTER(_vp)]),
    "kbbq_fastq_close": (None, [_vp]),
    "kbbq_fastq_num_reads": (_i64, [_vp]),
    "kbbq_fastq_read_len": (_i, [_vp]),
    "kbbq_fastq_pack": (_i, [_vp, _i64, _i64, _vp, _vp, _i]),
    "kbbq_fastq_name": (_i, [_vp, _i64, C.POINTER(C.c_char_p), C.POINTER(_i)]),
    "kbbq_fastq_infer": (_i, [_vp, _i, _vp, _vp, C.POINTER(_i), _i]),
    "kbbq_fastq_rg_key": (_i, [_vp, _i, C.POINTER(C.c_char_p), C.POINTER(_i)]),
    "kbbq_fastq_check_names": (_i, [_vp, _vp, _i64, _i, C.POINTER(_i64)]),
    "kbbq_fastq_write": (_i, [_i, _vp, _i64, _i64, _vp, _i]),
    "kbbq_fastq_format_size": (_i, [_vp, _i64, _i64, _i, C.POINTER(_i64)]),
    "kbbq_fastq_format": (_i, [_vp, _i64, _i64, _vp, _vp, _i64, _i]),
    "kbbq_host_mismatch_bits": (_i, [_vp, _vp, _i64, _vp, _i]),
    "kbbq_expand_mismatch_bits": (_i, [_vp, _vp, _i64, _vp, _vp]),
    "kbbq_host_last_traffic": (_i, [_i, C.POINTER(_i64), C.POINTER(_i64)]),
    "kbbq_host_pack_mode": (_i, [_i]),
    "kbbq_host_pack_nibbles": (_i, [_vp, _vp, _i64, _vp, _i, _vp]),
    "kbbq_expand_nibbles": (_i, [_vp, _i64, _vp, _vp, _vp]),
    "kbbq_plan_info": (_i, [_i, _i, _i, _i, _i, C.POINTER(_i)]),
    "kbbq_segment_rows_bound": (_i64, [_i64, _i]),
    "kbbq_segment_table_elems": (_i64, [_i]),
    "kbbq_segmented_supported": (_i, [_i, _i, _i]),
    "kbbq_segment_plan": (_i, [_vp, _vp, _i64, _i, _vp, _vp, _vp, _vp]),
    "kbbq_segment_rows": (_i, [_vp, _vp, _i64, _i, _vp, _vp]),
    "kbbq_segment_pad": (_i, [_vp, _i, _i, _vp, _vp, _vp, _vp]),
    "kbbq_unsegment_rows": (_i, [_vp, _vp, _i64, _i, _i64, _vp, _vp]),
    "kbbq_build_segmented": (_i, [_vp] * 4 + [_i64, _i, _i, _i] + [_vp] * 4 + [_vp, _sz, _vp, _vp]),
    "kbbq_apply_segmented": (_i, [_vp] * 3 + [_i64, _i, _i, _i] + [_vp] * 5 + [_i, _i, _vp, _vp, _sz, _vp, _vp]),
    "kbbq_apply_segmented_flags": (_i, [_vp] * 3 + [_i64, _i, _i, _i] + [_vp] * 5 + [_i, _i, _vp, _vp, _sz, _vp, _i, _vp]),
    "kbbq_kmer_table_bytes": (_i, [_i64, _i, _i, C.POINTER(C.c_uint64), C.POINTER(_sz)]),
    "kbbq_kmer_clear": (_i, [_vp, C.c_uint64, _vp]),
    "kbbq_kmer_count": (_i, [_vp, _i64, _i, _i, _vp, C.c_uint64, _vp, _vp]),
    "kbbq_kmer_histogram": (_i, [_vp, C.c_uint64, _vp, _vp]),
    "kbbq_kmer_flag": (_i, [_vp, _i64, _i, _i, _vp, C.c_uint64, _i, _vp, _vp, _vp]),
    "kbbq_kmer_min_count": (_i, [_vp]),
    "kbbq_kmer_errors_host": (_i, [_vp, _i64, _i, _i, _i, _vp, _vp, C.POINTER(_i), _i]),
    "kbbq_recalibrate_kmer_host": (_i, [_vp] * 4 + [_i64, _i, _i, _i, _i, _i] + [_vp] * 3 + [C.POINTER(_i), C.POINTER(_i), _i]),
}


class KbbqNativeError(RuntimeError):
    """The CUDA library is missing, or a CUDA / argument error came back from it."""


def lib():
    global _lib
    if _lib is None:
        if not os.path.exists(LIB_PATH):
            raise KbbqNativeError(
                "%s not found: build it with `python -c 'import __graft_entry__ as g; g.build()'` "
                "(or make -C kbbq-py_b200/csrc). kbbq_b200 has no CPU fallback." % LIB_PATH)
        handle = C.CDLL(LIB_PATH)
        for name, (res, args) in SIGNATURES.items():
            fn = getattr(handle, name)
            fn.restype = res
            fn.argtypes = args
        _lib = handle
    return _lib


def check(rc, status=0):
    if rc == 0:
        return
    if rc == E_DATA:
        raise_for_status(status)
    L = lib()
    msg = L.kbbq_strerror(rc).decode()
    if rc == -2:
        msg += ": " + L.kbbq_last_cuda_error().decode()
    raise KbbqNativeError("libkbbq_b200: %s (%d)" % (msg, rc))


def raise_for_status(status):
    if status & FLAG_QUAL_RANGE:
        raise IndexError("quality score out of range for the covariate tables (max 42)")
    if status & FLAG_BAD_BASE:
        raise TypeError("sequence contains a base outside A, C, G, T, N")
    if status & FLAG_RG_RANGE:
        raise IndexError("read group index out of range")
    if status & FLAG_SEGMENTS:
        raise ValueError("malformed span table of a segmented batch")
    if status & FLAG_KMER_FULL:
        raise MemoryError("the k-mer table is full")


def ptr(a):
    if a is None:
        return None
    assert a.flags["C_CONTIGUOUS"]
    return a.ctypes.data_as(C.c_void_p)


def u8(a):
    return np.ascontiguousarray(a, dtype=np.uint8)


def i64(a):
    return np.ascontiguousarray(a, dtype=np.int64)


def _opt(a, dtype=np.uint8):
    return None if a is None else np.ascontiguousarray(a, dtype=dtype)


def plan_info(L, R=1, minscore=6, arrays=3, max_smem=0):
    out = (C.c_int * 10)()
    if lib().kbbq_plan_info(L, R, minscore, arrays, max_smem, out) != 0:
        return None
    keys = ("G", "lanes", "ng", "threads", "nprod", "kps", "stages", "drep", "smem", "table_bytes")
    return dict(zip(keys, out))


DEVICE = int(os.environ.get("KBBQ_DEVICE", os.environ.get("LOCAL_RANK", "0")))


def _dev(device):
    return DEVICE if device is None else int(device)



def build_host(seq, qual, corr, rg, second, L, R, minscore=6, device=None):
    seq, qual, corr = u8(seq).ravel(), u8(qual).ravel(), u8(corr).ravel()
    N = seq.size // L
    assert seq.size == qual.size == corr.size == N * L
    rg = _opt(rg, np.uint16)
    second = _opt(second)
    pe, pt = np.zeros((R, NQ, 2 * L), np.int64), np.zeros((R, NQ, 2 * L), np.int64)
    de, dt = np.zeros((R, NQ, 16), np.int64), np.zeros((R, NQ, 16), np.int64)
    st = C.c_int(0)
    rc = lib().kbbq_build_host(ptr(seq), ptr(qual), ptr(corr), ptr(rg), ptr(second), N, L, R, minscore,
                               ptr(pe), ptr(pt), ptr(de), ptr(dt), C.byref(st), _dev(device))
    check(rc, st.value)
    return pe, pt, de, dt


def marginals_host(pos_errs, pos_total, device=None):
    pos_errs, pos_total = i64(pos_errs), i64(pos_total)
    R, nq, L2 = pos_total.shape
    assert nq == NQ
    q_e, q_t = np.zeros((R, NQ), np.int64), np.zeros((R, NQ), np.int64)
    g_e, g_t, mq = np.zeros(R, np.int64), np.zeros(R, np.int64), np.zeros(R, np.int64)
    check(lib().kbbq_marginals_host(ptr(pos_errs), ptr(pos_total), L2 // 2, R, ptr(q_e), ptr(q_t),
                                    ptr(g_e), ptr(g_t), ptr(mq), _dev(device)))
    return mq, g_e, g_t, q_e, q_t


def delta_q_host(prior_q, numerrs, numtotal, device=None):
    prior_q, numerrs, numtotal = i64(prior_q), i64(numerrs), i64(numtotal)
    out = np.zeros(prior_q.shape, np.int64)
    check(lib().kbbq_delta_q_host(ptr(prior_q), ptr(numerrs), ptr(numtotal), prior_q.size, ptr(out), _dev(device)))
    return out


def posterior_q_real_host(prior_q, numerrs, numtotal, device=None):
    prior_q = np.ascontiguousarray(prior_q, dtype=np.float64)
    numerrs, numtotal = i64(numerrs), i64(numtotal)
    out = np.zeros(prior_q.shape, np.int64)
    check(lib().kbbq_posterior_q_real_host(ptr(prior_q), ptr(numerrs), ptr(numtotal), prior_q.size, ptr(out),
                                           _dev(device)))
    return out


def calibration_counts_host(qual, err=None, seq=None, corr=None, skip=None, device=None):
    qual = u8(qual).ravel()
    arrs = [_opt(a) for a in (err, seq, corr, skip)]
    for a in arrs:
        assert a is None or a.size == qual.size
    total, errs = np.zeros(256, np.int64), np.zeros(256, np.int64)
    check(lib().kbbq_calibration_counts_host(ptr(qual), *[ptr(a) for a in arrs], qual.size, ptr(total), ptr(errs),
                                             _dev(device)))
    return total, errs


def build_bam_host(seq, qual, err, skip, rg, flags, aln_start, aln_end, L, R, minscore=6, tables=None, device=None):
    seq, qual, err = u8(seq).ravel(), u8(qual).ravel(), u8(err).ravel()
    skip = _opt(skip)
    N = seq.size // L
    assert seq.size == qual.size == err.size == N * L
    flags = _opt(flags)
    rg, aln_start, aln_end = _opt(rg, np.uint16), _opt(aln_start, np.uint16), _opt(aln_end, np.uint16)
    if tables is None:
        tables = (np.zeros((R, NQ, 2 * L), np.int64), np.zeros((R, NQ, 2 * L), np.int64),
                  np.zeros((R, NQ, 16), np.int64), np.zeros((R, NQ, 16), np.int64))
    pe, pt, de, dt = tables
    st = C.c_int(0)
    rc = lib().kbbq_build_bam_host(ptr(seq), ptr(qual), ptr(err), ptr(skip), ptr(rg), ptr(flags), ptr(aln_start),
                                   ptr(aln_end), N, L, R, minscore, ptr(pe), ptr(pt), ptr(de), ptr(dt), C.byref(st),
                                   _dev(device))
    check(rc, st.value)
    return pe, pt, de, dt


def apply_bam_host(seq, qual, rg, flags, L, R, meanq, rgdq, qdq, posdq, dindq, minscore=6, device=None):
    seq, qual = u8(seq).ravel(), u8(qual).ravel()
    N = seq.size // L
    flags = _opt(flags)
    rg = _opt(rg, np.uint16)
    meanq, rgdq, qdq, posdq, dindq = [i64(a) for a in (meanq, rgdq, qdq, posdq, dindq)]
    nq, ndin1 = qdq.shape[1], dindq.shape[2]
    assert posdq.shape == (R, nq, 2 * L) and dindq.shape[:2] == (R, nq)
    out = np.zeros((N, L), np.uint8)
    st = C.c_int(0)
    rc = lib().kbbq_apply_bam_host(ptr(seq), ptr(qual), ptr(rg), ptr(flags), N, L, R, minscore, ptr(meanq), ptr(rgdq),
                                   ptr(qdq), ptr(posdq), ptr(dindq), nq, ndin1, ptr(out), C.byref(st), _dev(device))
    check(rc, st.value)
    return out


def get_delta_qs_host(meanq, rg_errs, rg_total, q_errs, q_total, pos_errs, pos_total, din_errs, din_total,
                      device=None):
    arrs = [i64(a) for a in (meanq, rg_errs, rg_total, q_errs, q_total, pos_errs, pos_total, din_errs, din_total)]
    R, nq = arrs[4].shape
    ncyc, ndin = arrs[6].shape[2], arrs[8].shape[2]
    rgdq, qdq = np.zeros(R, np.int64), np.zeros((R, nq), np.int64)
    posdq, dindq = np.zeros((R, nq, ncyc), np.int64), np.zeros((R, nq, ndin + 1), np.int64)
    check(lib().kbbq_get_delta_qs_host(*[ptr(a) for a in arrs], R, nq, ncyc, ndin, ptr(rgdq), ptr(qdq),
                                       ptr(posdq), ptr(dindq), _dev(device)))
    return rgdq, qdq, posdq, dindq


def apply_host(seq, qual, rg, second, L, R, meanq, rgdq, qdq, posdq, dindq, minscore=6, device=None):
    seq, qual = u8(seq).ravel(), u8(qual).ravel()
    N = seq.size // L
    rg = _opt(rg, np.uint16)
    second = _opt(second)
    meanq, rgdq, qdq, posdq, dindq = [i64(a) for a in (meanq, rgdq, qdq, posdq, dindq)]
    nq, ndin1 = qdq.shape[1], dindq.shape[2]
    assert posdq.shape == (R, nq, 2 * L) and dindq.shape[:2] == (R, nq)
    out = np.zeros((N, L), np.uint8)
    st = C.c_int(0)
    rc = lib().kbbq_apply_host(ptr(seq), ptr(qual), ptr(rg), ptr(second), N, L, R, minscore, ptr(meanq),
                               ptr(rgdq), ptr(qdq), ptr(posdq), ptr(dindq), nq, ndin1, ptr(out),
                               C.byref(st), _dev(device))
    check(rc, st.value)
    return out


def device_list(devices=None):
    if devices is None:
        env = os.environ.get("KBBQ_DEVICES", "").strip()
        devices = [int(x) for x in env.split(",") if x.strip() != ""] if env else [DEVICE]
    elif isinstance(devices, int):
        devices = [devices]
    devices = [int(d) for d in devices]
    if not devices:
        raise ValueError("empty device list")
    return devices


# ... 190 lines not shown
```

kbbq-py_b200/kbbq/device.py:

```python
import ctypes as C
import weakref

import torch

from . import _native
from . import parallel

NQ = _native.NQ


def _p(t):
    return None if t is None else C.c_void_p(t.data_ptr())


def _on_device(fn):
    import functools

    @functools.wraps(fn)
    def wrapper(self, *args, **kwargs):
        with torch.cuda.device(self.device):
            return fn(self, *args, **kwargs)
    return wrapper


class SegmentedBatch:

    def __init__(self, seq, qual, corr, seg, dest, n_reads, rows_bound):
        self.seq, self.qual, self.corr, self.seg, self.dest = seq, qual, corr, seg, dest
        self.N, self.rows_bound = n_reads, rows_bound


class DeviceRecalibrator:

    def __init__(self, L, R=1, max_reads=0, minscore=6, device=None, process_group=None):
        if not torch.cuda.is_available():
            raise _native.KbbqNativeError("no CUDA device: kbbq_b200 has no CPU fallback")
        self.lib = _native.lib()
        self.L, self.R, self.minscore = int(L), int(R), int(minscore)
        self.device = torch.device("cuda", torch.cuda.current_device()) if device is None else torch.device(device)
        self.pg = process_group
        npos, ndin = R * NQ * 2 * L, R * NQ * 16
        with torch.cuda.device(self.device):
            self.tables = torch.zeros(2 * npos + 2 * ndin, dtype=torch.int64, device=self.device)
            self.pos_errs = self.tables[:npos].view(R, NQ, 2 * L)
            self.pos_total = self.tables[npos:2 * npos].view(R, NQ, 2 * L)
            self.din_errs = self.tables[2 * npos:2 * npos + ndin].view(R, NQ, 16)
            self.din_total = self.tables[2 * npos + ndin:].view(R, NQ, 16)
            self.q_errs = torch.zeros(R, NQ, dtype=torch.int64, device=self.device)
            self.q_total = torch.zeros(R, NQ, dtype=torch.int64, device=self.device)
            self.rg_errs = torch.zeros(R, dtype=torch.int64, device=self.device)
            self.rg_total = torch.zeros(R, dtype=torch.int64, device=self.device)
            self.meanq = torch.zeros(R, dtype=torch.int64, device=self.device)
            self.rgdq = torch.zeros(R, dtype=torch.int64, device=self.device)
            self.qdq = torch.zeros(R, NQ, dtype=torch.int64, device=self.device)
            self.posdq = torch.zeros(R, NQ, 2 * L, dtype=torch.int64, device=self.device)
            self.dindq = torch.zeros(R, NQ, 17, dtype=torch.int64, device=self.device)
            self.status = torch.zeros(1, dtype=torch.int32, device=self.device)
        self.workspace = None
        self.ws_reads = -1
        self._ensure_workspace(max_reads)
        self._built = []

    @_on_device
    def _ensure_workspace(self, n_reads):
        if n_reads <= self.ws_reads:
            return
        nbytes = C.c_size_t(0)
        _native.check(self.lib.kbbq_workspace_bytes(n_reads, self.L, self.R, C.byref(nbytes)))
        self.workspace = torch.empty(max(nbytes.value, 256), dtype=torch.uint8, device=self.device)
        self.ws_bytes = nbytes.value
        self.ws_reads = n_reads

    def _stream(self):
        return C.c_void_p(torch.cuda.current_stream(self.device).cuda_stream)

    def reset(self):
        self.tables.zero_()
        self.status.zero_()
        self._built = []

    @staticmethod
    def _version(t):
        try:
            return t._version
        except RuntimeError:
            return None

    def _remember_built(self, seq):
        v = self._version(seq)
        self._built = [(r, w) for r, w in self._built if r() is not None and r() is not seq]
        if v is not None:
            self._built.append((weakref.ref(seq), v))

    def _bases_checked(self, seq):
        v = self._version(seq)
        return v is not None and any(r() is seq and w == v for r, w in self._built)

    @_on_device
    def build(self, seq, qual, corr, rg=None, second=None, path=0):
        N = seq.numel() // self.L
        self._ensure_workspace(N)
        rc = self.lib.kbbq_build(_p(seq), _p(qual), _p(corr), _p(rg), _p(second), N, self.L, self.R, self.minscore,
                                 _p(self.pos_errs), _p(self.pos_total), _p(self.din_errs), _p(self.din_total),
                                 _p(self.workspace), self.ws_bytes, _p(self.status), path, self._stream())
        _native.check(rc)
        self._remember_built(seq)

    @_on_device
    def build_from_bits(self, seq, qual, bits, corr_scratch, rg=None, second=None):
        _native.check(self.lib.kbbq_expand_mismatch_bits(_p(seq), _p(bits), seq.numel(), _p(corr_scratch), self._stream()))
        self.build(seq, qual, corr_scratch, rg, second)

    @_on_device
    def segment(self, seq, qual, corr=None, rg=None, second=None):
        N, L, R = seq.numel() // self.L, self.L, self.R
        if not self.lib.kbbq_segmented_supported(L, R, self.minscore):
            raise _native.KbbqNativeError("no shared-memory plan for L=%d, R=%d: use build() / apply()" % (L, R))
        rows = int(self.lib.kbbq_segment_rows_bound(N, R))
        dev, st = self.device, self._stream()
        seg = torch.empty(int(self.lib.kbbq_segment_table_elems(R)), dtype=torch.int32, device=dev)
        dest = torch.empty(max(N, 1), dtype=torch.int32, device=dev)
        _native.check(self.lib.kbbq_segment_plan(_p(rg), _p(second), N, R, _p(seg), _p(dest), _p(self.status), st))
        outs = []
        for src in (seq, qual, corr):
            if src is None:
                outs.append(None)
                continue
            dst = torch.empty(rows * L + 16, dtype=torch.uint8, device=dev)
            _native.check(self.lib.kbbq_segment_rows(_p(src), _p(dest), N, L, _p(dst), st))
            outs.append(dst)
        _native.check(self.lib.kbbq_segment_pad(_p(seg), R, L, _p(outs[0]), _p(outs[1]), _p(outs[2]), st))
        return SegmentedBatch(outs[0], outs[1], outs[2], seg, dest, N, rows)

    @_on_device
    def build_segmented(self, sb):
        self._ensure_workspace(sb.rows_bound)
        rc = self.lib.kbbq_build_segmented(_p(sb.seq), _p(sb.qual), _p(sb.corr), _p(sb.seg), sb.rows_bound, self.L, self.R,
                                           self.minscore, _p(self.pos_errs), _p(self.pos_total), _p(self.din_errs),
                                           _p(self.din_total), _p(self.workspace), self.ws_bytes, _p(self.status),
                                           self._stream())
        _native.check(rc)
        self._remember_built(sb.seq)

    @_on_device
    def apply_segmented(self, sb, out_seg):
        self._ensure_workspace(sb.rows_bound)
        flags = _native.APPLY_BASES_CHECKED if self._bases_checked(sb.seq) else 0
        rc = self.lib.kbbq_apply_segmented_flags(_p(sb.seq), _p(sb.qual), _p(sb.seg), sb.rows_bound, self.L, self.R,
                                                 self.minscore, _p(self.meanq), _p(self.rgdq), _p(self.qdq),
                                                 _p(self.posdq), _p(self.dindq), NQ, 17, _p(out_seg), _p(self.workspace),
                                                 self.ws_bytes, _p(self.status), flags, self._stream())
        _native.check(rc)

    @_on_device
    def unsegment(self, sb, out_seg, out):
        _native.check(self.lib.kbbq_unsegment_rows(_p(out_seg), _p(sb.dest), sb.N, self.L, sb.rows_bound, _p(out),
                                                   self._stream()))

    def allreduce(self):
        parallel.allreduce_tables(self.tables, self.pg)

    @_on_device
    def model(self):
        L, R = self.L, self.R
        _native.check(self.lib.kbbq_marginals(_p(self.pos_errs), _p(self.pos_total), L, R, _p(self.q_errs),
                                              _p(self.q_total), _p(self.rg_errs), _p(self.rg_total),
                                              _p(self.meanq), self._stream()))
        _native.check(self.lib.kbbq_get_delta_qs(_p(self.meanq), _p(self.rg_errs), _p(self.rg_total),
                                                 _p(self.q_errs), _p(self.q_total), _p(self.pos_errs),
                                                 _p(self.pos_total), _p(self.din_errs), _p(self.din_total),
                                                 R, NQ, 2 * L, 16, _p(self.rgdq), _p(self.qdq), _p(self.posdq),
                                                 _p(self.dindq), self._stream()))

    @_on_device
    def apply(self, seq, qual, out, rg=None, second=None, path=0):
        N = seq.numel() // self.L
        self._ensure_workspace(N)
        if self._bases_checked(seq):
            path |= _native.APPLY_BASES_CHECKED
        rc = self.lib.kbbq_apply(_p(seq), _p(qual), _p(rg), _p(second), N, self.L, self.R, self.minscore,
                                 _p(self.meanq), _p(self.rgdq), _p(self.qdq), _p(self.posdq), _p(self.dindq),
                                 NQ, 17, _p(out), _p(self.workspace), self.ws_bytes, _p(self.status), path,
                                 self._stream())
        _native.check(rc)

    @_on_device
    def build_bam(self, seq, qual, err, skip=None, rg=None, flags=None, aln_start=None, aln_end=None, fast=True):
        N = seq.numel() // self.L
        ws = self._bam_workspace(N) if fast else None
        rc = self.lib.kbbq_build_bam(_p(seq), _p(qual), _p(err), _p(skip), _p(rg), _p(flags), _p(aln_start),
                                     _p(aln_end), N, self.L, self.R, self.minscore, _p(self.pos_errs),
                                     _p(self.pos_total), _p(self.din_errs), _p(self.din_total), _p(ws),
                                     0 if ws is None else ws.numel(), _p(self.status), self._stream())
        _native.check(rc)

    @_on_device
    def _bam_workspace(self, n_reads):
        if n_reads > getattr(self, "bam_ws_reads", -1):
            nbytes = C.c_size_t(0)
            _native.check(self.lib.kbbq_bam_workspace_bytes(n_reads, self.L, self.R, C.byref(nbytes)))
            self.bam_ws = torch.empty(max(nbytes.value, 256), dtype=torch.uint8, device=self.device)
            self.bam_ws_reads = n_reads
        return self.bam_ws

    @_on_device
    def apply_bam(self, seq, qual, out, rg=None, flags=None, fast=True):
        N = seq.numel() // self.L
        ws = self._bam_workspace(N) if fast else None
        rc = self.lib.kbbq_apply_bam(_p(seq), _p(qual), _p(rg), _p(flags), N, self.L, self.R, self.minscore,
                                     _p(self.meanq), _p(self.rgdq), _p(self.qdq), _p(self.posdq), _p(self.dindq),
                                     NQ, 17, _p(out), _p(ws), 0 if ws is None else ws.numel(), _p(self.status),
                                     self._stream())
        _native.check(rc)

    @_on_device
    def check_status(self):
        st = int(self.status.item())
        if st:
            _native.raise_for_status(st)

    def covariate_arrays(self):
        self.model()
        return tuple(t.cpu().numpy().copy() for t in (self.meanq, self.rg_errs, self.rg_total, self.q_errs,
                                                      self.q_total, self.pos_errs, self.pos_total,
                                                      self.din_errs, self.din_total))

    def delta_qs(self):
        return tuple(t.cpu().numpy().copy() for t in (self.rgdq, self.qdq, self.posdq, self.dindq))


def calibration_counts(qual, err=None, seq=None, corr=None, skip=None, total=None, errs=None):
    lib = _native.lib()
    dev = qual.device
    torch.cuda.set_device(dev)
    if total is None:
        total = torch.zeros(256, dtype=torch.int64, device=dev)
    if errs is None:
        errs = torch.zeros(256, dtype=torch.int64, device=dev)
    rc = lib.kbbq_calibration_counts(_p(qual), _p(err), _p(seq), _p(corr), _p(skip), qual.numel(), _p(total),
                                     _p(errs), C.c_void_p(torch.cuda.current_stream(dev).cuda_stream))
    _native.check(rc)
    return total, errs


def synth_reads(seed, first_read, n, L, R, device=None, want_corr=True):
    lib = _native.lib()
    dev = torch.device("cuda", torch.cuda.current_device()) if device is None else torch.device(device)
    torch.cuda.set_device(dev)
    seq = torch.empty(n, L, dtype=torch.uint8, device=dev)
    qual = torch.empty(n, L, dtype=torch.uint8, device=dev)
    corr = torch.empty(n, L, dtype=torch.uint8, device=dev)
    rg = torch.empty(n, dtype=torch.int16, device=dev)
    second = torch.empty(n, dtype=torch.uint8, device=dev)
    rc = lib.kbbq_synth_reads(seed, first_read, n, L, R, _p(seq), _p(qual), _p(corr), _p(rg), _p(second),
                              C.c_void_p(torch.cuda.current_stream(dev).cuda_stream))
    _native.check(rc)
    return seq, qual, corr, rg, second
```

Baseline: 869.1 billion.

## Reuse build-time prepare in apply and parallelize model kernels across warp lanes

Apply now skips re-running the read-group/segment prepare step (uniform memset and prep kernels) when the preceding build used the same workspace and the same rg/second/seg arrays. This is tracked with a host-side mark list and Python tensor version checks. The model kernels change too: marginals are fused into one kernel for short reads, posterior search is split across several lanes per cell with the constant tables staged in shared memory, and lane counts are sized to SM residency. The cost is added cache-validity bookkeeping, which risks stale state if the workspace contents are changed between build and apply.

After: 893.6 billion (median of 6 runs). 2.8% higher.

```diff
diff --git a/include/kbbq_b200.h b/include/kbbq_b200.h
--- a/include/kbbq_b200.h
+++ b/include/kbbq_b200.h
@@ -83,6 +83,7 @@
                       void *stream);
 
 #define KBBQ_APPLY_BASES_CHECKED 0x10
+#define KBBQ_APPLY_PREPARED 0x20
 int kbbq_apply(const uint8_t *seq_dev, const uint8_t *qual_dev, const uint16_t *rg_dev,
                const uint8_t *second_dev, int64_t N, int L, int R, int minscore,
                const int64_t *meanq_dev, const int64_t *rgdq_dev, const int64_t *qdq_dev,
diff --git a/kbbq-py_b200/csrc/host_api.cu b/kbbq-py_b200/csrc/host_api.cu
--- a/kbbq-py_b200/csrc/host_api.cu
+++ b/kbbq-py_b200/csrc/host_api.cu
@@ -1429,7 +1429,7 @@
     KBBQ_TRY(kbbq_get_delta_qs(mp.meanq, mp.rg_errs, mp.rg_total, mp.q_errs, mp.q_total, pe, pt, de, dt, R, NQ, 2 * L,
                                16, mp.rgdq, mp.qdq, mp.posdq, mp.dindq, nullptr));
     KBBQ_TRY(kbbq_apply(d_seq, d_qual, d_rg, d_sec, N, L, R, minscore, mp.meanq, mp.rgdq, mp.qdq, mp.posdq, mp.dindq, NQ,
-                        17, d_out, ws, ws_bytes, c.status, KBBQ_APPLY_BASES_CHECKED, nullptr));
+                        17, d_out, ws, ws_bytes, c.status, KBBQ_APPLY_BASES_CHECKED | KBBQ_APPLY_PREPARED, nullptr));
     if (tables_host) KBBQ_CUDA(cudaMemcpy(tables_host, pe, ntab * 8, cudaMemcpyDeviceToHost));
     if (deltas_host)
         KBBQ_CUDA(cudaMemcpy(deltas_host, mp.meanq, ((size_t)2 * R + (size_t)R * NQ * (1 + 2 * L + 17)) * 8,
diff --git a/kbbq-py_b200/csrc/kbbq_b200.cu b/kbbq-py_b200/csrc/kbbq_b200.cu
--- a/kbbq-py_b200/csrc/kbbq_b200.cu
+++ b/kbbq-py_b200/csrc/kbbq_b200.cu
@@ -52,6 +52,21 @@
     if (*sms <= 0) *sms = KBBQ_SM_COUNT_FALLBACK;
     if (*device < 64) { s_smem[*device].store(*max_smem); s_sms[*device].store(*sms); }
     return KBBQ_OK;
+}
+
+constexpr int MODEL_THREADS = 256;
+constexpr long long MODEL_RESIDENT_PER_SM = 1536;
+static int model_lanes_log2(long long cells, int *lw) {
+    int device, sms, max_smem;
+    int rc = current_device_info(&device, &sms, &max_smem);
+    if (rc) return rc;
+    const long long resident = (long long)sms * MODEL_RESIDENT_PER_SM;
+    *lw = 0;
+    while (*lw < 5 && (cells << (*lw + 1)) <= resident) ++*lw;
+    return KBBQ_OK;
+}
+static unsigned int model_blocks(long long cells, int lw) {
+    return (unsigned int)(((cells << lw) + MODEL_THREADS - 1) / MODEL_THREADS);
 }
 
 static bool misaligned(const void *p, size_t a) { return ((uintptr_t)p & (a - 1)) != 0; }
@@ -121,6 +136,31 @@
     return KBBQ_OK;
 }
 
+struct PrepMark {
+    const void *ws, *rg, *second, *seg_rows;
+    int64_t N;
+    int G, R;
+    bool operator==(const PrepMark &o) const {
+        return ws == o.ws && rg == o.rg && second == o.second && seg_rows == o.seg_rows && N == o.N && G == o.G && R == o.R;
+    }
+};
+static std::mutex g_prep_mu;
+static std::vector<PrepMark> g_prep;
+static void prep_forget(const void *ws) {
+    std::lock_guard<std::mutex> lock(g_prep_mu);
+    g_prep.erase(std::remove_if(g_prep.begin(), g_prep.end(), [&](const PrepMark &m) { return m.ws == ws; }), g_prep.end());
+}
+static void prep_remember(const PrepMark &m) {
+    prep_forget(m.ws);
+    std::lock_guard<std::mutex> lock(g_prep_mu);
+    if (g_prep.size() >= 64) g_prep.erase(g_prep.begin());
+    g_prep.push_back(m);
+}
+static bool prep_remembered(const PrepMark &m) {
+    std::lock_guard<std::mutex> lock(g_prep_mu);
+    return std::find(g_prep.begin(), g_prep.end(), m) != g_prep.end();
+}
+
 struct SmemPlan {
     Geom g;
     TableCfg tc;
@@ -134,7 +174,8 @@
 template <class Generic>
 static int plan_and_prepare(int narr, bool aligned, int64_t N, int L, int R, int minscore, const uint16_t *rg,
                             const uint8_t *second, void *workspace, size_t workspace_bytes, int *status, int path,
-                            const unsigned int *seg_rows, cudaStream_t st, const Generic &generic, SmemPlan *p) {
+                            const unsigned int *seg_rows, bool prepared, cudaStream_t st, const Generic &generic,
+                            SmemPlan *p) {
     const bool segmode = seg_rows != nullptr;
     int device, max_smem;
     int rc = current_device_info(&device, &p->sms, &max_smem);
@@ -143,23 +184,29 @@
               (uint64_t)((N + p->g.G - 1) / p->g.G) < 0xFFFFFFFFull;
     if (!p->smem) {
         if (path == 1 || segmode) return KBBQ_E_ARG;
+        if (narr == 3 && workspace) prep_forget(workspace);
         return generic(0, N, p->sms * 8);
     }
     p->w = carve_workspace(workspace, N, L, R);
     if (!workspace || workspace_bytes < p->w.bytes) return KBBQ_E_WORKSPACE;
     p->N = N;
+    const int64_t tail = (!segmode && R == 1 && N > p->g.G) ? N % p->g.G : 0;
+    const PrepMark mark = {workspace, rg, second, seg_rows, N - tail, p->g.G, R};
+    const bool reuse = narr == 2 && prepared && (segmode || R == 1) && prep_remembered(mark);
+    if (narr == 3) prep_remember(mark);
+    else if (!reuse) prep_forget(workspace);
     if (segmode) {
+        if (reuse) return KBBQ_OK;
         seg_prepare_kernel<<<1, 256, 0, st>>>(seg_rows, 2 * R, p->g.G, (unsigned long long)N, p->w.seg, p->w.uni, status);
         KBBQ_LAUNCHED();
         return KBBQ_OK;
     }
-    const int64_t tail = (R == 1 && N > p->g.G) ? N % p->g.G : 0;
     if (tail) {
         p->N = N - tail;
         rc = generic(p->N, tail, 1);
         if (rc) return rc;
     }
-    return run_prepare(rg, second, p->N, p->g.G, R, p->w, status, p->sms, p->sl.ngs, p->g.gbytes, p->sl.slot, st);
+    return run_prepare(rg, second, p->N, p->g.G, R, p->w, status, p->sms, p->sl.ngs, p->g.gbytes, p->sl.slot, reuse, st);
 }
 
 template <class Launch>
@@ -249,7 +296,7 @@
     const bool aligned = !misaligned(seq, 16) && !misaligned(qual, 16) && !misaligned(corr, 16);
     SmemPlan p;
     int rc = plan_and_prepare(3, aligned, N, L, R, minscore, rg, second, workspace, workspace_bytes, status, path,
-                              seg_rows, st, generic, &p);
+                              seg_rows, false, st, generic, &p);
     if (rc || !p.smem) return rc;
 
     BuildArgs a;
@@ -287,11 +334,16 @@
     cudaStream_t st = (cudaStream_t)stream;
     int rc = upload_constants();
     if (rc) return rc;
-    marginals_q_kernel<<<dim3(NQ, R), 128, 0, st>>>((const long long *)pos_errs, (const long long *)pos_total,
-                                                   2 * L, (long long *)q_errs, (long long *)q_total);
-    KBBQ_LAUNCHED();
-    marginals_rg_kernel<<<R, 64, 0, st>>>((const long long *)q_errs, (const long long *)q_total, R,
-                                                      (long long *)rg_errs, (long long *)rg_total, (long long *)meanq);
+    const bool split = 2 * L > MARGINALS_ONE_BLOCK_L2;
+    if (split) {
+        marginals_q_kernel<<<dim3(NQ, R), 128, 0, st>>>((const long long *)pos_errs, (const long long *)pos_total, 2 * L,
+                                                       (long long *)q_errs, (long long *)q_total);
+        KBBQ_LAUNCHED();
+    }
+    marginals_kernel<<<R, MARGINALS_THREADS, 0, st>>>(split ? nullptr : (const long long *)pos_errs,
+                                                      (const long long *)pos_total, 2 * L,
+                                                      (long long *)q_errs, (long long *)q_total, (long long *)rg_errs,
+                                                      (long long *)rg_total, (long long *)meanq);
     KBBQ_LAUNCHED();
     return KBBQ_OK;
 }
@@ -302,8 +354,11 @@
     if (n == 0) return KBBQ_OK;
     int rc = upload_constants();
     if (rc) return rc;
-    delta_q_kernel<<<(unsigned)((n + 127) / 128), 128, 0, (cudaStream_t)stream>>>(
-        (const long long *)prior_q, (const long long *)numerrs, (const long long *)numtotal, n, (long long *)delta);
+    int lw;
+    rc = model_lanes_log2(n, &lw);
+    if (rc) return rc;
+    delta_q_kernel<<<model_blocks(n, lw), MODEL_THREADS, 0, (cudaStream_t)stream>>>(
+        (const long long *)prior_q, (const long long *)numerrs, (const long long *)numtotal, n, lw, (long long *)delta);
     KBBQ_LAUNCHED();
     return KBBQ_OK;
 }
@@ -314,8 +369,11 @@
     if (n == 0) return KBBQ_OK;
     int rc = upload_constants();
     if (rc) return rc;
-    posterior_q_real_kernel<<<(unsigned)((n + 127) / 128), 128, 0, (cudaStream_t)stream>>>(
-        prior_q, (const long long *)numerrs, (const long long *)numtotal, n, (long long *)posterior);
+    int lw;
+    rc = model_lanes_log2(n, &lw);
+    if (rc) return rc;
+    posterior_q_real_kernel<<<model_blocks(n, lw), MODEL_THREADS, 0, (cudaStream_t)stream>>>(
+        prior_q, (const long long *)numerrs, (const long long *)numtotal, n, lw, (long long *)posterior);
     KBBQ_LAUNCHED();
     return KBBQ_OK;
 }
@@ -473,10 +531,13 @@
                    (const long long *)q_errs, (const long long *)q_total, (const long long *)pos_errs,
                    (const long long *)pos_total, (const long long *)din_errs, (const long long *)din_total,
                    R, nq, ncyc, ndin, (long long *)rgdq, (long long *)qdq, (long long *)posdq, (long long *)dindq};
-    delta_levels12_kernel<<<R, 64, 0, st>>>(a);
-    KBBQ_LAUNCHED();
     const long long cells = (long long)R * nq * (ncyc + ndin + 1);
-    delta_level3_kernel<<<(unsigned)((cells + 127) / 128), 128, 0, st>>>(a);
+    int lw;
+    rc = model_lanes_log2(cells, &lw);
+    if (rc) return rc;
+    delta_levels12_kernel<<<R, LEVELS12_THREADS, 0, st>>>(a);
+    KBBQ_LAUNCHED();
+    delta_level3_kernel<<<model_blocks(cells, lw), MODEL_THREADS, 0, st>>>(a, lw);
     KBBQ_LAUNCHED();
     return KBBQ_OK;
 }
@@ -488,7 +549,8 @@
                       const unsigned int *seg_rows) {
     const bool segmode = seg_rows != nullptr;
     const bool validate = !(path & KBBQ_APPLY_BASES_CHECKED);
-    path &= ~KBBQ_APPLY_BASES_CHECKED;
+    const bool prepared = (path & KBBQ_APPLY_PREPARED) != 0;
+    path &= ~(KBBQ_APPLY_BASES_CHECKED | KBBQ_APPLY_PREPARED);
     if (N < 0 || L < 1 || R < 1 || R > 65535 || minscore < 0 || minscore >= NQ) return KBBQ_E_ARG;
     if (nq < 1 || nq > NQ || ndin1 < 16 || ndin1 > 64) return KBBQ_E_ARG;
     if (!meanq || !rgdq || !qdq || !posdq || !dindq || !status) return KBBQ_E_ARG;
@@ -514,7 +576,7 @@
     const bool aligned = !misaligned(seq, 16) && !misaligned(qual, 16) && !misaligned(out_qual, 4);
     SmemPlan p;
     int rc = plan_and_prepare(2, aligned, N, L, R, minscore, rg, second, workspace, workspace_bytes, status, path,
-                              seg_rows, st, generic, &p);
+                              seg_rows, prepared, st, generic, &p);
     if (rc || !p.smem) return rc;
 
     ApplyArgs a;
@@ -537,7 +599,7 @@
                                int R, int minscore, const int64_t *meanq, const int64_t *rgdq, const int64_t *qdq,
                                const int64_t *posdq, const int64_t *dindq, int nq, int ndin1, uint8_t *out_qual,
                                void *workspace, size_t workspace_bytes, int *status, int flags, void *stream) {
-    if (!seg || rows_bound % SEG_ALIGN || (flags & ~KBBQ_APPLY_BASES_CHECKED)) return KBBQ_E_ARG;
+    if (!seg || rows_bound % SEG_ALIGN || (flags & ~(KBBQ_APPLY_BASES_CHECKED | KBBQ_APPLY_PREPARED))) return KBBQ_E_ARG;
     return apply_impl(seq, qual, nullptr, nullptr, rows_bound, L, R, minscore, meanq, rgdq, qdq, posdq, dindq, nq, ndin1,
                       out_qual, workspace, workspace_bytes, status, 1 | flags, stream, seg);
 }
diff --git a/kbbq-py_b200/csrc/model.cuh b/kbbq-py_b200/csrc/model.cuh
--- a/kbbq-py_b200/csrc/model.cuh
+++ b/kbbq-py_b200/csrc/model.cuh
@@ -36,6 +36,17 @@
     return a.hi < bh || (a.hi == bh && a.lo <= bl);
 }
 
+struct ModelTables { double lnp[NQ], ln1mp[NQ], prior[NQ]; };
+__device__ __forceinline__ void load_model_tables(ModelTables &t) {
+    for (int i = threadIdx.x; i < NQ; i += blockDim.x) {
+        t.lnp[i] = c_lnp[i];
+        t.ln1mp[i] = c_ln1mp[i];
+        t.prior[i] = c_prior[i];
+    }
+    __syncthreads();
+}
+
+constexpr int MARGINALS_ONE_BLOCK_L2 = 1024;
 __global__ void marginals_q_kernel(const long long *pos_errs, const long long *pos_total, int L2,
                                    long long *q_errs, long long *q_total) {
     const int q = blockIdx.x, rg = blockIdx.y;
@@ -54,35 +65,63 @@
     }
 }
 
-__global__ void marginals_rg_kernel(const long long *q_errs, const long long *q_total, int R,
-                                    long long *rg_errs, long long *rg_total, long long *meanq) {
-    const int rg = blockIdx.x;
+constexpr int MARGINALS_THREADS = 1024;
+__global__ void __launch_bounds__(MARGINALS_THREADS) marginals_kernel(const long long *pos_errs, const long long *pos_total,
+                                                                      int L2, long long *q_errs, long long *q_total,
+                                                                      long long *rg_errs, long long *rg_total,
+                                                                      long long *meanq) {
+    const int rg = blockIdx.x, lane = threadIdx.x & 31;
     __shared__ long long s_e[NQ], s_t[NQ];
-    if (threadIdx.x < NQ) {
-        s_e[threadIdx.x] = q_errs[rg * NQ + threadIdx.x];
-        s_t[threadIdx.x] = q_total[rg * NQ + threadIdx.x];
-    }
-    __syncthreads();
-    if (threadIdx.x != 0) return;
-    long long e = 0, t = 0;
-    dd acc = {0.0, 0.0};
-    for (int q = 0; q < NQ; ++q) {
-        const long long tq = s_t[q];
-        e += s_e[q];
-        t += tq;
-        if (tq) acc = dd_add(acc, two_prod((double)tq, c_p[q]));
-    }
-    rg_errs[rg] = e;
-    rg_total[rg] = t;
-    long long mq = 0;
-    if (t > 0) {
-        if (acc.hi == 0.0) mq = NQ - 1;
-        else {
-            const dd p = dd_div_d(acc, (double)t);
-            for (int m = 1; m < NQ; ++m) mq += dd_le(p, c_bound_hi[m], c_bound_lo[m]) ? 1 : 0;
-        }
-    }
-    meanq[rg] = mq;
+    __shared__ dd s_p;
+    __shared__ int s_live;
+    for (int q = threadIdx.x >> 5; q < NQ; q += blockDim.x >> 5) {
+        if (!pos_errs) {
+            if (lane == 0) {
+                s_e[q] = q_errs[rg * NQ + q];
+                s_t[q] = q_total[rg * NQ + q];
+            }
+            continue;
+        }
+        const size_t base = ((size_t)rg * NQ + q) * L2;
+        long long e = 0, t = 0;
+        for (int c0 = lane; c0 < L2; c0 += 8 * 32) {
+            long long ev[8], tv[8];
+#pragma unroll
+            for (int u = 0; u < 8; ++u) {
+                const int c = c0 + 32 * u;
+                ev[u] = c < L2 ? pos_errs[base + c] : 0;
+                tv[u] = c < L2 ? pos_total[base + c] : 0;
+            }
+#pragma unroll
+            for (int u = 0; u < 8; ++u) { e += ev[u]; t += tv[u]; }
+        }
+        for (int o = 16; o; o >>= 1) { e += __shfl_down_sync(0xFFFFFFFFu, e, o); t += __shfl_down_sync(0xFFFFFFFFu, t, o); }
+        if (lane == 0) {
+            s_e[q] = e;
+            s_t[q] = t;
+            q_errs[rg * NQ + q] = e;
+            q_total[rg * NQ + q] = t;
+        }
+    }
+    __syncthreads();
+    if (threadIdx.x == 0) {
+        long long e = 0, t = 0;
+        dd acc = {0.0, 0.0};
+        for (int q = 0; q < NQ; ++q) {
+            const long long tq = s_t[q];
+            e += s_e[q];
+            t += tq;
+            if (tq) acc = dd_add(acc, two_prod((double)tq, c_p[q]));
+        }
+        rg_errs[rg] = e;
+        rg_total[rg] = t;
+        s_live = t > 0 ? (acc.hi == 0.0 ? 2 : 1) : 0;
+        if (s_live == 1) s_p = dd_div_d(acc, (double)t);
+    }
+    __syncthreads();
+    const int m = threadIdx.x;
+    const int below = __syncthreads_count(s_live == 1 && m >= 1 && m < NQ && dd_le(s_p, c_bound_hi[m], c_bound_lo[m]));
+    if (threadIdx.x == 0) meanq[rg] = s_live == 0 ? 0 : s_live == 2 ? NQ - 1 : below;
 }
 
 __device__ __forceinline__ dd round_to_x87(dd s) {
@@ -98,39 +137,57 @@
 }
 
 template <typename PRIOR>
-__device__ __forceinline__ int posterior_q_cell(PRIOR prior, long long errs, long long tot) {
+__device__ __forceinline__ dd posterior_candidate(const ModelTables &t, PRIOR prior, double k, double mm, int c) {
+    int d = (int)((PRIOR)c - prior);
+    d = d < 0 ? -d : d;
+    const double pr = d < NQ ? t.prior[d] : -KBBQ_INF;
+    const double a = __dmul_rn(k, t.lnp[c]);
+    const double b = (mm == 0.0) ? 0.0 : __dmul_rn(mm, t.ln1mp[c]);
+    const double ll = __dadd_rn(a, b);
+    if (isinf(pr) || isinf(ll)) return {-KBBQ_INF, 0.0};
+    return round_to_x87(two_sum(pr, ll));
+}
+
+template <typename PRIOR>
+__device__ __forceinline__ int posterior_q_cell(const ModelTables &t, PRIOR prior, long long errs, long long tot, int j,
+                                                int W) {
     const double k = (double)(errs + 1), mm = (double)((tot + 2) - (errs + 1));
-    int best = 0;
-    double bh = 0.0, bl = 0.0;
-    bool have = false;
-    for (int c = 0; c < NQ; ++c) {
-        int d = (int)((PRIOR)c - prior);
-        d = d < 0 ? -d : d;
-        const double pr = d < NQ ? c_prior[d] : -KBBQ_INF;
-        const double a = __dmul_rn(k, c_lnp[c]);
-        const double b = (mm == 0.0) ? 0.0 : __dmul_rn(mm, c_ln1mp[c]);
-        const double ll = __dadd_rn(a, b);
-        double h, l;
-        if (isinf(pr) || isinf(ll)) { h = -KBBQ_INF; l = 0.0; }
-        else { dd s = round_to_x87(two_sum(pr, ll)); h = s.hi; l = s.lo; }
-        if (!have || h > bh || (h == bh && l > bl)) { best = c; bh = h; bl = l; have = true; }
+    int best = j;
+    dd b = posterior_candidate(t, prior, k, mm, j);
+    for (int c = j + W; c < NQ; c += W) {
+        const dd s = posterior_candidate(t, prior, k, mm, c);
+        if (s.hi > b.hi || (s.hi == b.hi && s.lo > b.lo)) { best = c; b = s; }
+    }
+    const unsigned int mask = W == 32 ? 0xFFFFFFFFu : ((1u << W) - 1u) << ((threadIdx.x & 31) & ~(W - 1));
+    for (int o = W >> 1; o; o >>= 1) {
+        const double oh = __shfl_xor_sync(mask, b.hi, o), ol = __shfl_xor_sync(mask, b.lo, o);
+        const int oc = __shfl_xor_sync(mask, best, o);
+        if (oh > b.hi || (oh == b.hi && (ol > b.lo || (ol == b.lo && oc < best)))) { best = oc; b = {oh, ol}; }
     }
     return best;
 }
-__device__ __forceinline__ int delta_q_cell(int prior, long long errs, long long tot) {
-    return posterior_q_cell<int>(prior, errs, tot) - prior;
-}
-
-__global__ void delta_q_kernel(const long long *prior, const long long *errs, const long long *tot,
-                               long long n, long long *out) {
-    long long i = (long long)blockIdx.x * blockDim.x + threadIdx.x;
-    if (i < n) out[i] = delta_q_cell((int)prior[i], errs[i], tot[i]);
-}
-
-__global__ void posterior_q_real_kernel(const double *prior, const long long *errs, const long long *tot,
-                                        long long n, long long *out) {
-    long long i = (long long)blockIdx.x * blockDim.x + threadIdx.x;
-    if (i < n) out[i] = posterior_q_cell<double>(prior[i], errs[i], tot[i]);
+
+__global__ void delta_q_kernel(const long long *prior, const long long *errs, const long long *tot, long long n, int lw,
+                               long long *out) {
+    __shared__ ModelTables s_t;
+    load_model_tables(s_t);
+    const long long t = (long long)blockIdx.x * blockDim.x + threadIdx.x, i = t >> lw;
+    const int W = 1 << lw, j = (int)(t & (W - 1));
+    if (i >= n) return;
+    const int p = (int)prior[i];
+    const int c = posterior_q_cell<int>(s_t, p, errs[i], tot[i], j, W);
+    if (j == 0) out[i] = c - p;
+}
+
+__global__ void posterior_q_real_kernel(const double *prior, const long long *errs, const long long *tot, long long n,
+                                        int lw, long long *out) {
+    __shared__ ModelTables s_t;
+    load_model_tables(s_t);
+    const long long t = (long long)blockIdx.x * blockDim.x + threadIdx.x, i = t >> lw;
+    const int W = 1 << lw, j = (int)(t & (W - 1));
+    if (i >= n) return;
+    const int c = posterior_q_cell<double>(s_t, prior[i], errs[i], tot[i], j, W);
+    if (j == 0) out[i] = c;
 }
 
 struct DeltaArgs {
@@ -139,37 +196,57 @@
     long long *rgdq, *qdq, *posdq, *dindq;
 };
 
-__global__ void delta_levels12_kernel(DeltaArgs a) {
+constexpr int LEVEL2_LANES = 16;
+constexpr int LEVELS12_THREADS = 704;
+__global__ void __launch_bounds__(LEVELS12_THREADS) delta_levels12_kernel(DeltaArgs a) {
+    __shared__ ModelTables s_t;
+    __shared__ int s_prior1;
+    load_model_tables(s_t);
     const int rg = blockIdx.x;
-    __shared__ int s_prior1;
-    if (threadIdx.x == 0) {
+    if (threadIdx.x < 32) {
         const int mq = (int)a.meanq[rg];
-        const int d = delta_q_cell(mq, a.rg_errs[rg], a.rg_total[rg]);
-        a.rgdq[rg] = d;
-        s_prior1 = mq + d;
-    }
-    __syncthreads();
-    for (int q = threadIdx.x; q < a.nq; q += blockDim.x)
-        a.qdq[rg * a.nq + q] = delta_q_cell(s_prior1, a.q_errs[rg * a.nq + q], a.q_total[rg * a.nq + q]);
-}
-
-__global__ void delta_level3_kernel(DeltaArgs a) {
+        const int d = posterior_q_cell<int>(s_t, mq, a.rg_errs[rg], a.rg_total[rg], threadIdx.x, 32) - mq;
+        if (threadIdx.x == 0) {
+            a.rgdq[rg] = d;
+            s_prior1 = mq + d;
+        }
+    }
+    __syncthreads();
+    const int j = threadIdx.x & (LEVEL2_LANES - 1);
+    for (int q = threadIdx.x / LEVEL2_LANES; q < a.nq; q += blockDim.x / LEVEL2_LANES) {
+        const long long i = (long long)rg * a.nq + q;
+        const int d = posterior_q_cell<int>(s_t, s_prior1, a.q_errs[i], a.q_total[i], j, LEVEL2_LANES) - s_prior1;
+        if (j == 0) a.qdq[i] = d;
+    }
+}
+
+__global__ void delta_level3_kernel(DeltaArgs a, int lw) {
+    __shared__ ModelTables s_t;
+    load_model_tables(s_t);
     const long long ncell_pos = (long long)a.R * a.nq * a.ncyc;
     const long long ncell_din = (long long)a.R * a.nq * (a.ndin + 1);
-    long long i = (long long)blockIdx.x * blockDim.x + threadIdx.x;
+    const long long t = (long long)blockIdx.x * blockDim.x + threadIdx.x;
+    const int W = 1 << lw, j = (int)(t & (W - 1));
+    long long i = t >> lw;
     if (i < ncell_pos) {
         const long long gq = i / a.ncyc;
         const int rg = (int)(gq / a.nq);
         const int prior2 = (int)(a.meanq[rg] + a.rgdq[rg] + a.qdq[gq]);
-        a.posdq[i] = delta_q_cell(prior2, a.pos_errs[i], a.pos_total[i]);
+        const int d = posterior_q_cell<int>(s_t, prior2, a.pos_errs[i], a.pos_total[i], j, W) - prior2;
+        if (j == 0) a.posdq[i] = d;
     } else if (i < ncell_pos + ncell_din) {
         i -= ncell_pos;
         const long long gq = i / (a.ndin + 1);
-        const int d = (int)(i - gq * (a.ndin + 1));
-        if (d == a.ndin) { a.dindq[i] = 0; return; }
+        const int dn = (int)(i - gq * (a.ndin + 1));
+        if (dn == a.ndin) {
+            if (j == 0) a.dindq[i] = 0;
+            return;
+        }
         const int rg = (int)(gq / a.nq);
         const int prior2 = (int)(a.meanq[rg] + a.rgdq[rg] + a.qdq[gq]);
-        a.dindq[i] = delta_q_cell(prior2, a.din_errs[gq * a.ndin + d], a.din_total[gq * a.ndin + d]);
+        const long long c = gq * a.ndin + dn;
+        const int d = posterior_q_cell<int>(s_t, prior2, a.din_errs[c], a.din_total[c], j, W) - prior2;
+        if (j == 0) a.dindq[i] = d;
     }
 }
 
diff --git a/kbbq-py_b200/csrc/prepare.cuh b/kbbq-py_b200/csrc/prepare.cuh
--- a/kbbq-py_b200/csrc/prepare.cuh
+++ b/kbbq-py_b200/csrc/prepare.cuh
@@ -259,13 +259,13 @@
 
 inline int run_prepare(const uint16_t *rg, const uint8_t *second, long long N, int G, int R,
                        const Workspace &w, int *status, int grid, int ng, unsigned int gbytes,
-                       unsigned int slot, cudaStream_t st) {
+                       unsigned int slot, bool uniform_done, cudaStream_t st) {
     PrepArgs a;
     a.rg = rg; a.second = second; a.N = N; a.G = G;
     a.ngroups = (N + G - 1) / G; a.R = R;
     a.seg = w.seg; a.cursor = w.cursor; a.entries = w.entries; a.uni = w.uni; a.status = status;
     a.grid = grid; a.ng = ng; a.gbytes = gbytes; a.slot = slot;
-    KBBQ_CUDA(cudaMemsetAsync(w.uni, (R == 1 && a.ngroups > 0) ? 0 : 0xFF, sizeof(unsigned int) * 4, st));
+    if (!uniform_done) KBBQ_CUDA(cudaMemsetAsync(w.uni, (R == 1 && a.ngroups > 0) ? 0 : 0xFF, sizeof(unsigned int) * 4, st));
     if (a.ngroups == 0) {
         KBBQ_CUDA(cudaMemsetAsync(w.seg, 0, sizeof(unsigned int) * ((size_t)R + 1), st));
         return KBBQ_OK;
@@ -273,8 +273,10 @@
     const unsigned int blocks = (unsigned int)((a.ngroups + PREP_THREADS - 1) / PREP_THREADS);
     if (R == 1) {
         const unsigned int few = std::min<unsigned int>(blocks, (unsigned int)std::max(grid, 1) * 8u);
-        prep_uniform_kernel<<<few, PREP_THREADS, 0, st>>>(a);
-        KBBQ_LAUNCHED();
+        if (!uniform_done) {
+            prep_uniform_kernel<<<few, PREP_THREADS, 0, st>>>(a);
+            KBBQ_LAUNCHED();
+        }
         prep_identity_kernel<<<few, PREP_THREADS, 0, st>>>(a);
         KBBQ_LAUNCHED();
         return KBBQ_OK;
diff --git a/kbbq-py_b200/kbbq/_native.py b/kbbq-py_b200/kbbq/_native.py
--- a/kbbq-py_b200/kbbq/_native.py
+++ b/kbbq-py_b200/kbbq/_native.py
@@ -10,6 +10,7 @@
 FLAG_QUAL_RANGE, FLAG_BAD_BASE, FLAG_RG_RANGE, FLAG_SEGMENTS = 1, 2, 4, 8
 FLAG_KMER_FULL = 16
 APPLY_BASES_CHECKED = 0x10
+APPLY_PREPARED = 0x20
 E_DATA = -4
 E_UNSUPPORTED = -12
 
diff --git a/kbbq-py_b200/kbbq/device.py b/kbbq-py_b200/kbbq/device.py
--- a/kbbq-py_b200/kbbq/device.py
+++ b/kbbq-py_b200/kbbq/device.py
@@ -58,6 +58,7 @@
             self.status = torch.zeros(1, dtype=torch.int32, device=self.device)
         self.workspace = None
         self.ws_reads = -1
+        self._prepared = None
         self._ensure_workspace(max_reads)
         self._built = []
 
@@ -70,6 +71,7 @@
         self.workspace = torch.empty(max(nbytes.value, 256), dtype=torch.uint8, device=self.device)
         self.ws_bytes = nbytes.value
         self.ws_reads = n_reads
+        self._prepared = None
 
     def _stream(self):
         return C.c_void_p(torch.cuda.current_stream(self.device).cuda_stream)
@@ -78,6 +80,7 @@
         self.tables.zero_()
         self.status.zero_()
         self._built = []
+        self._prepared = None
 
     @staticmethod
     def _version(t):
@@ -92,6 +95,25 @@
         if v is not None:
             self._built.append((weakref.ref(seq), v))
 
+    def _arrays_mark(self, *ts):
+        mark = []
+        for t in ts:
+            v = None if t is None else self._version(t)
+            if t is not None and v is None:
+                return None
+            mark.append(None if t is None else (weakref.ref(t), v))
+        return tuple(mark)
+
+    def _take_prepared(self, *ts):
+        mark, self._prepared = self._prepared, None
+        if mark is None or len(mark) != len(ts):
+            return False
+        for m, t in zip(mark, ts):
+            if (m is None) != (t is None) or (t is not None and (m[0]() is not t or m[1] != self._version(t))):
+                return False
+        self._prepared = mark
+        return True
+
     def _bases_checked(self, seq):
         v = self._version(seq)
         return v is not None and any(r() is seq and w == v for r, w in self._built)
@@ -103,8 +125,10 @@
         rc = self.lib.kbbq_build(_p(seq), _p(qual), _p(corr), _p(rg), _p(second), N, self.L, self.R, self.minscore,
                                  _p(self.pos_errs), _p(self.pos_total), _p(self.din_errs), _p(self.din_total),
                                  _p(self.workspace), self.ws_bytes, _p(self.status), path, self._stream())
+        self._prepared = None
         _native.check(rc)
         self._remember_built(seq)
+        self._prepared = self._arrays_mark(rg, second)
 
     @_on_device
     def build_from_bits(self, seq, qual, bits, corr_scratch, rg=None, second=None):
@@ -139,13 +163,17 @@
                                            self.minscore, _p(self.pos_errs), _p(self.pos_total), _p(self.din_errs),
                                            _p(self.din_total), _p(self.workspace), self.ws_bytes, _p(self.status),
                                            self._stream())
+        self._prepared = None
         _native.check(rc)
         self._remember_built(sb.seq)
+        self._prepared = self._arrays_mark(sb.seg)
 
     @_on_device
     def apply_segmented(self, sb, out_seg):
         self._ensure_workspace(sb.rows_bound)
         flags = _native.APPLY_BASES_CHECKED if self._bases_checked(sb.seq) else 0
+        if self._take_prepared(sb.seg):
+            flags |= _native.APPLY_PREPARED
         rc = self.lib.kbbq_apply_segmented_flags(_p(sb.seq), _p(sb.qual), _p(sb.seg), sb.rows_bound, self.L, self.R,
                                                  self.minscore, _p(self.meanq), _p(self.rgdq), _p(self.qdq),
                                                  _p(self.posdq), _p(self.dindq), NQ, 17, _p(out_seg), _p(self.workspace),
@@ -178,6 +206,8 @@
         self._ensure_workspace(N)
         if self._bases_checked(seq):
             path |= _native.APPLY_BASES_CHECKED
+        if self._take_prepared(rg, second):
+            path |= _native.APPLY_PREPARED
         rc = self.lib.kbbq_apply(_p(seq), _p(qual), _p(rg), _p(second), N, self.L, self.R, self.minscore,
                                  _p(self.meanq), _p(self.rgdq), _p(self.qdq), _p(self.posdq), _p(self.dindq),
                                  NQ, 17, _p(out), _p(self.workspace), self.ws_bytes, _p(self.status), path,
```
